# antrea-io/theia

Measured on AMD Instinct MI355X. Metric: flow-records/sec, higher is better.
Workload: dtype u64 (aggregates) + f64 (detectors)

## Files before the change

theia_amd/csrc/tad_capi.cpp:

```cpp
#include "tad_engine.h"

using namespace tad;
using namespace tadh;

namespace tadh {

int ensure_rcp_table(JobCtx *e, uint64_t T) {
  const uint64_t want = T + 2;
  if (want <= e->rcp_n) return TAD_OK;
  uint64_t cap = want < 1024 ? 1024 : want + want / 4;
  int rc = ensure(e, e->rcp_table, cap * sizeof(double));
  if (rc != TAD_OK) return rc;
  std::vector<double> h(cap);
  h[0] = 0.0;
  for (uint64_t i = 1; i < cap; ++i) h[i] = 1.0 / (double)i;
  HIP_TRY(e, hipMemcpyAsync(e->rcp_table.p, h.data(), cap * sizeof(double), hipMemcpyHostToDevice, e->stream));
  HIP_TRY(e, hipStreamSynchronize(e->stream));
  e->rcp_n = cap;
  return TAD_OK;
}

int ensure_key_buffers(JobCtx *e, uint64_t K) {
  int rc;
  const uint64_t k = K ? K : 1;
  if ((rc = ensure(e, e->sigma, k * sizeof(double))) != TAD_OK) return rc;
  if ((rc = ensure(e, e->n_pts, k * sizeof(uint32_t))) != TAD_OK) return rc;
  if ((rc = ensure(e, e->n_anom, k * sizeof(uint32_t))) != TAD_OK) return rc;
  if ((rc = ensure(e, e->off, (k + 1) * sizeof(unsigned long long))) != TAD_OK) return rc;
  if ((rc = ensure(e, e->scan_scratch, scan_scratch_elems(k) * sizeof(unsigned long long))) != TAD_OK) return rc;
  if ((rc = ensure(e, e->key_mean, k * sizeof(double))) != TAD_OK) return rc;
  if ((rc = ensure(e, e->key_m2, k * sizeof(double))) != TAD_OK) return rc;
  if ((rc = ensure(e, e->counters, kTailBytes)) != TAD_OK) return rc;
  return TAD_OK;
}

void emit_rows(JobCtx *e, Grid g, Lattice L, const JobParams &jp, OutRows out, uint64_t rows) {
  const int kind = jp.algo == TAD_ALGO_EWMA ? 0 : (jp.algo == TAD_ALGO_ARIMA ? 1 : (jp.algo == TAD_ALGO_DROP ? 3 : (jp.lazy_sigma ? 4 : 2)));
  if (kind == 4 && !jp.all_points &&
      launch_emit_dbscan_list(e->stream, g, L, e->aux.p, static_cast<const uint32_t *>(e->n_anom.p), static_cast<const unsigned long long *>(e->off.p), out))
    return;
  launch_emit(e->stream, g, L, kind, jp.all_points, jp.alpha, static_cast<const double *>(e->sigma.p),
              static_cast<const uint32_t *>(e->n_pts.p), static_cast<const double *>(kind == 3 ? e->key_mean.p : e->calc.p),
              static_cast<const unsigned long long *>(e->off.p), out, rows, e->plan.ewma_emit, e->plan.ewma_emit_rows);
}

int make_result(JobCtx *e, uint64_t rows, bool with_anomaly, tad_mem out_memory, ResultPriv **out, OutRows *dev_rows,
                ResultBlock *dev_block) {
  ResultPriv *rp = new (std::nothrow) ResultPriv();
  if (!rp) return fail(e, TAD_ERR_OUT_OF_MEMORY, "out of host memory");
  memset(rp, 0, sizeof *rp);
  const size_t bytes = result_bytes(rows, with_anomaly);
  int rc = alloc_device_block(e, bytes, dev_block);
  if (rc != TAD_OK) { delete rp; return rc; }
  carve(dev_block->base, rows, with_anomaly, dev_rows);
  rp->pub.n_rows = rows;
  rp->pub.memory = out_memory;
  *out = rp;
  return TAD_OK;
}

int finish_result(JobCtx *e, ResultPriv *rp, uint64_t rows, bool with_anomaly, ResultBlock dev_block, OutRows dev_rows) {
  if (rp->pub.memory == TAD_MEM_DEVICE) {
    rp->block = dev_block.base;
    rp->block_cap = dev_block.cap;
    rp->pub.key_id = reinterpret_cast<uint64_t *>(dev_rows.key_id);
    rp->pub.flow_end_s = reinterpret_cast<int64_t *>(dev_rows.flow_end_s);
    rp->pub.throughput = dev_rows.throughput;
    rp->pub.algo_calc = dev_rows.algo_calc;
    rp->pub.stddev = dev_rows.stddev;
    rp->pub.anomaly = dev_rows.anomaly;
    return TAD_OK;
  }
  const size_t bytes = result_bytes(rows, with_anomaly);
  void *h = malloc(bytes);
  if (!h) { release_block(e, dev_block.base, dev_block.cap); return fail(e, TAD_ERR_OUT_OF_MEMORY, "out of host memory for %zu result bytes", bytes); }
  hipError_t r = hipMemcpyAsync(h, dev_block.base, bytes, hipMemcpyDeviceToHost, e->stream);
  if (r == hipSuccess) r = hipStreamSynchronize(e->stream);
  release_block(e, dev_block.base, dev_block.cap);
  if (r != hipSuccess) { free(h); return fail(e, TAD_ERR_HIP, "result copy failed: %s", hipGetErrorString(r)); }
  OutRows ho;
  carve(h, rows, with_anomaly, &ho);
  rp->block = h;
  rp->block_cap = bytes;
  rp->pub.key_id = reinterpret_cast<uint64_t *>(ho.key_id);
  rp->pub.flow_end_s = reinterpret_cast<int64_t *>(ho.flow_end_s);
  rp->pub.throughput = ho.throughput;
  rp->pub.algo_calc = ho.algo_calc;
  rp->pub.stddev = ho.stddev;
  rp->pub.anomaly = ho.anomaly;
  return TAD_OK;
}

JobParams job_params(const tad_job *job) {
  JobParams jp;
  jp.algo = job->algo;
  jp.alpha = job->ewma_alpha == 0.0 ? 0.5 : job->ewma_alpha;
  jp.eps = job->dbscan_eps == 0.0 ? 250000000.0 : job->dbscan_eps;
  jp.min_samples = job->dbscan_min_samples == 0 ? 4 : job->dbscan_min_samples;
  jp.maxiter = job->arima_maxiter == 0 ? 50 : job->arima_maxiter;
  jp.drop_nsigma = job->drop_nsigma == 0.0 ? 3.0 : job->drop_nsigma;
  jp.drop_min_samples = job->drop_min_samples == 0 ? 3 : job->drop_min_samples;
  jp.all_points = (job->flags & TAD_FLAG_EMIT_ALL_POINTS) != 0;
  return jp;
}

void merge_moments(const Moments *blocks, bool any, double *pts_mean, double *pts_m2) {
  double mn = 0.0, mean = 0.0, m2 = 0.0;
  if (any)
    for (int b = 0; b < kMomentBlocks; ++b) {
      const Moments &p = blocks[b];
      if (p.n == 0.0) continue;
      if (mn == 0.0) { mn = p.n; mean = p.mean; m2 = p.m2; continue; }
      const double nn = mn + p.n, d = p.mean - mean;
      mean = mean + d * (p.n / nn);
      m2 = m2 + p.m2 + d * d * (mn * p.n / nn);
      mn = nn;
    }
  *pts_mean = mean;
  *pts_m2 = m2;
}

static int count_verdicts(JobCtx *e, ResultPriv *rp, uint64_t rows, uint64_t *n_anomalies) {
  *n_anomalies = 0;
  if (rows == 0) return TAD_OK;
  std::vector<uint8_t> tmp;
  const uint8_t *a = rp->pub.anomaly;
// ... 433 lines not shown
```

theia_amd/csrc/tad_capi_job.cpp:

```cpp
#include "tad_engine.h"

using namespace tad;
using namespace tadh;

namespace {

struct Job {
  const tad_job *job;
  const tad_columns *cols;
  tad_state *stream;
  bool points_mode;
  int depth;
  tad_mem out_memory;
  JobParams jp;
  tad_plan plan;
  bool op_max, has2;
  uint64_t n, K, slots_all;
  RowFilter rf;
  int cw;
  const void *d_key, *d_key2, *d_te, *d_ts, *d_val;
  DevCounters *ctr;
  bool empty;
};

struct Attempt {
  bool retry = false;
  bool finished = false;
  bool hinted = false;
  PartPlan pl{};
  Lattice L{};
  Grid g{};
  uint64_t cells = 0, need = 0;
  bool cells_overflow = false;
  bool v2 = false, sparse = false, sp_part = false, hist_sampled = false, use_kh = false, narrow_tiles = false;
  const uint32_t *binhist = nullptr;
  const unsigned long long *stream_poff = nullptr;
  uint64_t stream_P = 0;
  int stage0_path() const { return sparse ? (sp_part ? 8 : 4) : (v2 ? (pl.wc_cap ? 3 : 2) : 1); }
  int hist_source() const { return (v2 && hist_sampled) ? 1 : (use_kh ? 2 : 0); }
};

int decide(JobCtx *e, const Job &j, Stage0Retry &rs, Attempt &a, Stage0Facts f) {
  f.v2 = a.v2; f.sparse = a.sparse; f.sp_part = a.sp_part; f.use_kh = a.use_kh; f.hist_sampled = a.hist_sampled; f.narrow_tiles = a.narrow_tiles;
  const Stage0Next x = rs.next(f);
  a.retry = x.what == Stage0Next::kRetry;
  if (x.what != Stage0Next::kFail) return TAD_OK;
  if (x.code == TAD_ERR_GRID_TOO_LARGE)
    return fail(e, x.code, x.msg, (unsigned long long)a.need, (unsigned long long)j.K, (unsigned long long)a.L.nb, (long long)a.L.step, (unsigned long long)e->ws_limit);
  return fail(e, x.code, x.msg, (unsigned long long)j.K);
}

int decide(JobCtx *e, const Job &j, Stage0Retry &rs, Attempt &a, uint32_t err) {
  Stage0Facts f;
  f.err = err;
  return decide(e, j, rs, a, f);
}

int detect_and_count(JobCtx *e, Grid g, JobParams &jp, DevCounters *ctr, uint64_t *rows) {
  hipStream_t s = e->stream;
  int rc;
  if ((rc = ensure_key_buffers(e, g.K)) != TAD_OK) return rc;
  if ((rc = ensure_rcp_table(e, g.T)) != TAD_OK) return rc;
  double *sigma = static_cast<double *>(e->sigma.p);
  uint32_t *n_pts = static_cast<uint32_t *>(e->n_pts.p);
  uint32_t *n_anom = static_cast<uint32_t *>(e->n_anom.p);
  unsigned long long *off = static_cast<unsigned long long *>(e->off.p);

  const bool ewma = jp.algo == TAD_ALGO_EWMA;
  const bool drop = jp.algo == TAD_ALGO_DROP;
  const bool db_fused = jp.algo == TAD_ALGO_DBSCAN && !jp.all_points && dbscan_uses_list(g);
  jp.lazy_sigma = db_fused;
  if (drop) {
    if ((rc = ensure(e, e->calc, (g.K * g.T ? g.K * g.T : 1) * sizeof(double))) != TAD_OK) return rc;
    launch_drop(s, g, jp.drop_nsigma, jp.drop_min_samples, static_cast<double *>(e->calc.p), sigma, n_pts,
                static_cast<double *>(e->key_mean.p), static_cast<double *>(e->key_m2.p), ctr);
  } else if (!db_fused)
    launch_key_sigma(s, g, jp.alpha, ewma && !jp.all_points, static_cast<const double *>(e->rcp_table.p), sigma, n_pts, n_anom, ctr, static_cast<double *>(e->key_mean.p),
                     static_cast<double *>(e->key_m2.p));
  if (jp.algo == TAD_ALGO_DBSCAN) {
    if ((rc = ensure(e, e->aux, dbscan_scratch_bytes(g))) != TAD_OK) return rc;
    if (dbscan_uses_list(g)) {
      DbscanStats dst{nullptr, nullptr, nullptr, nullptr};
      if (db_fused) dst = DbscanStats{n_pts, n_anom, static_cast<double *>(e->key_mean.p), static_cast<double *>(e->key_m2.p)};
      if (launch_dbscan(s, g, jp.eps, jp.min_samples, e->aux.p, dst, jp.settled && db_fused) != 0)
        return fail(e, TAD_ERR_HIP, "DBSCAN launch failed");
    } else {
      return fail(e, TAD_ERR_GRID_TOO_LARGE, "DBSCAN: series of %llu buckets are not supported", (unsigned long long)g.T);
    }
  } else if (jp.algo == TAD_ALGO_ARIMA) {
    if ((rc = ensure(e, e->calc, g.K * g.T * sizeof(double))) != TAD_OK) return rc;
    const size_t wsb = arima_workspace_bytes(g);
    if ((rc = ensure(e, e->aux, wsb)) != TAD_OK) return rc;
    const bool held = e->hold && e->hold->held;
    if (held) e->hold->release();
    const unsigned int *yielded_dev = nullptr;
    if (launch_arima(s, g, sigma, n_pts, jp.maxiter, static_cast<double *>(e->calc.p), ctr, e->aux.p, wsb, e->eng->pause_dev, &yielded_dev) != 0)
      return fail(e, TAD_ERR_HIP, "ARIMA launch failed");
    if ((rc = arima_yield_loop(e, yielded_dev, [&](uint32_t grace, const unsigned int **yd) {
           return launch_arima_fit(s, g, sigma, n_pts, jp.maxiter, static_cast<double *>(e->calc.p), ctr, e->aux.p, e->eng->pause_dev, yd, grace);
         })) != TAD_OK)
      return rc;
    if (held) e->hold->acquire();
  }
  const uint32_t *cnt = n_anom;
  if (jp.all_points && jp.algo != TAD_ALGO_ARIMA && !drop) cnt = n_pts;
  else if (db_fused) {}
  else if (!ewma || jp.all_points) launch_count_flags(s, g, jp.all_points, n_anom);
  launch_scan_moments(s, cnt, off, g.K, static_cast<unsigned long long *>(e->scan_scratch.p), dev_total(e), n_pts,
                      static_cast<const double *>(e->key_mean.p), static_cast<const double *>(e->key_m2.p), dev_moments(e), db_fused ? ctr : nullptr);
  HIP_TRY(e, hipMemcpyAsync(e->tail_host, e->counters.p, kTailBytes, hipMemcpyDeviceToHost, s));
  HIP_TRY(e, hipStreamSynchronize(s));
  HIP_TRY(e, hipGetLastError());
  *rows = *e->total_host;
  return TAD_OK;
}

int stage_column(JobCtx *e, DevBuf &buf, const void *src, uint64_t n, tad_mem mem, const void **dev, uint64_t width = 8) {
  if (!src) { *dev = nullptr; return TAD_OK; }
  if (mem == TAD_MEM_DEVICE) { *dev = src; return TAD_OK; }
  int rc = ensure(e, buf, n * width);
  if (rc != TAD_OK) return rc;
  HIP_TRY(e, hipMemcpyAsync(buf.p, src, n * width, hipMemcpyHostToDevice, e->stream));
  *dev = buf.p;
  return TAD_OK;
}

int stage_columns(JobCtx *e, Job &j) {
  const tad_columns *cols = j.cols;
  const uint64_t kw = (j.cw & kColKey32) ? 4 : 8, tw = (j.cw & kColTime32) ? 4 : 8;
  int rc;
  if ((rc = stage_column(e, e->in_key, cols->key_id, j.n, cols->memory, &j.d_key, kw)) != TAD_OK) return rc;
  if ((rc = stage_column(e, e->in_key2, cols->key_id2, j.n, cols->memory, &j.d_key2, kw)) != TAD_OK) return rc;
  if ((rc = stage_column(e, e->in_te, cols->flow_end_s, j.n, cols->memory, &j.d_te, tw)) != TAD_OK) return rc;
  if ((rc = stage_column(e, e->in_ts, cols->flow_start_s, j.n, cols->memory, &j.d_ts, tw)) != TAD_OK) return rc;
  return stage_column(e, e->in_val, cols->value, j.n, cols->memory, &j.d_val);
}


int pass_a(JobCtx *e, const Job &j, const Stage0Retry &rs, Attempt &a, int *meta_blocks) {
  hipStream_t s = e->stream;
  int rc;
  const uint64_t n = j.n, K = j.K;
  a.v2 = !j.empty && j.plan.stage0 != 1 && !rs.v1 && (j.plan.stage0 == 2 || n >= (1ull << 22)) && part_plan_bins(n, K, j.has2, &a.pl);
  if (a.v2 && e->hold) e->hold->acquire();
  if ((rc = ensure(e, e->meta, sizeof(MetaPartial) * kMetaBlocks)) != TAD_OK) return rc;
  *meta_blocks = 0;
  if (!a.v2) return TAD_OK;
  const PartPlan &pl = a.pl;
  const tad_key_hist *kh = j.cols->key_hist;
  a.use_kh = j.depth == 0 && !rs.kh_rejected && kh != nullptr && kh->bins != nullptr && rs.lat_mode != 2 && kh->n_rows == n && kh->num_keys == K &&
             kh->sides == (j.has2 ? 2u : 1u) && kh->workgroups == (uint32_t)pl.G && kh->nbins == pl.nbins && kh->shift == (uint32_t)pl.shift_bin &&
             kh->chunk_rows == pl.chunk && j.rf.end_time == 0 && !(j.d_ts != nullptr && j.rf.start_time != 0);
  if ((rc = ensure(e, e->binhist, (size_t)pl.G * pl.nbins * 4)) != TAD_OK) return rc;
  a.hist_sampled = launch_meta_hist(s, (const uint64_t *)j.d_key, (const uint64_t *)j.d_key2, (const int64_t *)j.d_te, (const int64_t *)j.d_ts, n, K, j.rf,
                                    pl, static_cast<MetaPartial *>(e->meta.p), static_cast<uint32_t *>(e->binhist.p), j.ctr, j.cw,
                                    a.use_kh ||
                                    (!rs.exact_hist && rs.lat_mode != 2 && sampled_slots_bound(j.slots_all, pl) < (1ull << 32) &&
                                        (j.plan.histogram == 2 ||
                                         j.slots_all / ((uint64_t)pl.G * ((K >> kSampleBlockShift) ? (K >> kSampleBlockShift) : 1)) >= 384)));
  *meta_blocks = pl.G;
  a.binhist = static_cast<const uint32_t *>(e->binhist.p);
// ... 200 lines not shown
                                 reinterpret_cast<const uint32_t *>(ss.uval), a.L.t0, a.g, static_cast<long long *>(e->sp_times.p));
    else
      launch_sparse_place(s, ss.ucomp, ss.uval, P, static_cast<const uint32_t *>(e->sp_first.p), a.L.t0, a.g, static_cast<long long *>(e->sp_times.p));
  }
  HIP_TRY(e, hipEventRecord(e->ev[3], s));
  return TAD_OK;
}

int stage0_sparse(JobCtx *e, const Job &j, Stage0Retry &rs, Attempt &a, tad_result **out, tad_points **points_out) {
  SparseSort ss;
  int rc;
  if ((rc = sparse_sort(e, j, rs, a, ss)) != TAD_OK || a.retry) return rc;
  if (j.stream) return sparse_stream_offsets(e, j, a, ss);
  return sparse_rank_grid(e, j, rs, a, ss, out, points_out);
}

int settle_setup(JobCtx *e, Job &j, const Stage0Retry &rs, Attempt &a, SettleArgs *settle, uint32_t **ovf_keys) {
  hipStream_t s = e->stream;
  const Grid g = a.g;
  int rc;
  *settle = SettleArgs{};
  *ovf_keys = nullptr;
  j.jp.settled = false;
  if (!(j.jp.algo == TAD_ALGO_DBSCAN && !j.jp.all_points && !j.points_mode && !j.stream && dbscan_uses_list(g) &&
        part_plan_settle(a.L.nb, &a.pl, j.op_max && !rs.wide_tiles)))
    return TAD_OK;
  if ((rc = ensure(e, e->aux, dbscan_scratch_bytes(g))) != TAD_OK) return rc;
  if ((rc = ensure(e, e->ovf_keys, ((size_t)(j.K + 31) / 32) * 4 + 64)) != TAD_OK) return rc;
  *ovf_keys = static_cast<uint32_t *>(e->ovf_keys.p);
  HIP_TRY(e, hipMemsetAsync(*ovf_keys, 0, ((size_t)(j.K + 31) / 32) * 4, s));
  unsigned int *cnt = static_cast<unsigned int *>(e->aux.p);
  HIP_TRY(e, hipMemsetAsync(cnt, 0, 2 * sizeof(unsigned int), s));
  settle->redo_list = dbscan_redo_list(g, e->aux.p);
  settle->redo_count = cnt + 1;
  settle->st = DbscanStats{static_cast<uint32_t *>(e->n_pts.p), static_cast<uint32_t *>(e->n_anom.p), static_cast<double *>(e->key_mean.p),
                           static_cast<double *>(e->key_m2.p)};
  settle->list = reinterpret_cast<uint32_t *>(static_cast<unsigned char *>(e->aux.p) + 64);
  settle->count = cnt;
  settle->eps = j.jp.eps;
  settle->min_samples = j.jp.min_samples;
  settle->on = 1;
  settle->ovf_keys = *ovf_keys;
  dbscan_compact_series(g, e->aux.p, &settle->cs_val, &settle->cs_flag, &settle->cs_has, &settle->cs_cap);
  dbscan_redo_series(g, e->aux.p, &settle->rs_val, &settle->rs_flag, &settle->rs_has, &settle->rs_cap);
  j.jp.settled = true;
  a.narrow_tiles = a.pl.narrow;
  return TAD_OK;
}

int stage0_tiles(JobCtx *e, Job &j, Stage0Retry &rs, Attempt &a) {
  hipStream_t s = e->stream;
  const uint64_t n = j.n, K = j.K;
  PartPlan &pl = a.pl;
  int rc;
  part_plan_wc(a.hist_sampled ? sampled_slots_bound(j.slots_all, pl) : j.slots_all, columns_aligned16(j.d_key, j.d_key2, j.d_te, j.d_val), j.has2, j.plan.partition_pass, &pl);
  const uint64_t slots = a.hist_sampled ? sampled_slots_bound(j.slots_all, pl) : j.slots_all + pl.pad_slots;
  {
    Stage0Facts f;
    f.sampled_slots_2_32 = a.hist_sampled && slots >= (1ull << 32);
    if ((rc = decide(e, j, rs, a, f)) != TAD_OK || a.retry) return rc;
  }
  uint32_t *fin = nullptr;
  if (a.hist_sampled) {
    if ((rc = ensure(e, e->part_fin, (size_t)pl.G * pl.nparts * 8)) != TAD_OK) return rc;
    fin = static_cast<uint32_t *>(e->part_fin.p);
  }
  if ((rc = ensure(e, e->part_total, (size_t)pl.nparts * 4)) != TAD_OK) return rc;
  if ((rc = ensure(e, e->part_start, ((size_t)pl.nparts + 1) * 8)) != TAD_OK) return rc;
  if ((rc = ensure(e, e->part_offs32, (size_t)pl.G * pl.nparts * 4)) != TAD_OK) return rc;
  if ((rc = ensure(e, e->recs, (size_t)slots * 8)) != TAD_OK) return rc;
  if ((rc = ensure(e, e->ovf, 16 + (size_t)kOverflowCap * sizeof(OverflowRec))) != TAD_OK) return rc;
  unsigned long long *ovf_count = dev_ovf_count(e);
  OverflowRec *ovf = reinterpret_cast<OverflowRec *>(static_cast<unsigned char *>(e->ovf.p) + 16);
  if ((rc = ensure_key_buffers(e, K)) != TAD_OK) return rc;
  if ((rc = ensure_rcp_table(e, a.L.nb)) != TAD_OK) return rc;
  uint32_t *offs32 = static_cast<uint32_t *>(e->part_offs32.p);
  unsigned long long *part_start = static_cast<unsigned long long *>(e->part_start.p);
  if ((rc = ensure(e, e->slices, slice_table_bytes(slots, pl))) != TAD_OK) return rc;
  launch_part_offsets(s, a.binhist, pl, offs32, static_cast<uint32_t *>(e->part_total.p), part_start,
                      a.hist_sampled, static_cast<const MetaPartial *>(e->meta.p), n, slots, e->slices.p, a.g, j.ctr);
  SettleArgs settle;
  uint32_t *ovf_keys;
  if ((rc = settle_setup(e, j, rs, a, &settle, &ovf_keys)) != TAD_OK) return rc;
  HIP_TRY(e, hipEventRecord(e->ev[2], s));
  launch_partition(s, (const uint64_t *)j.d_key, (const uint64_t *)j.d_key2, (const int64_t *)j.d_te, (const int64_t *)j.d_ts,
                   (const uint64_t *)j.d_val, n, K, j.rf, a.L, pl, offs32, part_start, e->recs.p, ovf, ovf_count, kOverflowCap, j.ctr, fin, ovf_keys, j.cw);
  HIP_TRY(e, hipEventRecord(e->ev[3], s));
  launch_tile_aggregate(s, e->recs.p, part_start, pl, slots, e->slices.p, a.g, j.op_max, ovf, ovf_count, kOverflowCap,
                        a.hist_sampled ? offs32 : nullptr, fin, settle);
  return TAD_OK;
}

int stage0_dense(JobCtx *e, Job &j, Stage0Retry &rs, Attempt &a) {
  hipStream_t s = e->stream;
  const uint64_t K = j.K;
  int rc;
  if (a.cells_overflow) return fail(e, TAD_ERR_GRID_TOO_LARGE, "grid of %llu keys x %llu buckets overflows", (unsigned long long)K, (unsigned long long)a.L.nb);
  {
    Stage0Facts f;
    f.grid_too_large = a.need > e->ws_limit;
    if ((rc = decide(e, j, rs, a, f)) != TAD_OK || a.retry) return rc;
  }
  if ((rc = ensure(e, e->grid_val, a.cells * 8)) != TAD_OK) return rc;
  if ((rc = ensure(e, e->grid_flag, a.cells)) != TAD_OK) return rc;
  a.g = Grid{static_cast<unsigned long long *>(e->grid_val.p), static_cast<uint8_t *>(e->grid_flag.p), j.empty ? 0 : K, a.L.nb, nullptr};
  if (a.v2 && !part_plan_tiles(K, a.L.nb, j.has2, &a.pl)) a.v2 = false;
  if (a.v2) return stage0_tiles(e, j, rs, a);
  if (a.cells) {
    HIP_TRY(e, hipMemsetAsync(a.g.val, 0, a.cells * 8, s));
    HIP_TRY(e, hipMemsetAsync(a.g.flag, 0, a.cells, s));
  }
  HIP_TRY(e, hipEventRecord(e->ev[2], s));
  if (!j.empty)
    launch_scatter(s, (const uint64_t *)j.d_key, (const uint64_t *)j.d_key2, (const int64_t *)j.d_te, (const int64_t *)j.d_ts,
                   (const uint64_t *)j.d_val, j.n, j.rf, a.L, a.g, j.op_max, j.ctr, j.cw);
  HIP_TRY(e, hipEventRecord(e->ev[3], s));
  return TAD_OK;
}


int count_points(JobCtx *e, const Job &j, const Attempt &a, uint64_t *rows) {
  hipStream_t s = e->stream;
  const Grid g = a.g;
  int rc;
  if ((rc = ensure_key_buffers(e, g.K)) != TAD_OK) return rc;
  if ((rc = ensure_rcp_table(e, g.T)) != TAD_OK) return rc;
  launch_key_sigma(s, g, 0.5, false, static_cast<const double *>(e->rcp_table.p), static_cast<double *>(e->sigma.p),
                   static_cast<uint32_t *>(e->n_pts.p), static_cast<uint32_t *>(e->n_anom.p), j.ctr, static_cast<double *>(e->key_mean.p),
                   static_cast<double *>(e->key_m2.p));
  launch_moments(s, g.K, static_cast<const uint32_t *>(e->n_pts.p), static_cast<const double *>(e->key_mean.p),
                 static_cast<const double *>(e->key_m2.p), dev_moments(e));
  unsigned long long *off = static_cast<unsigned long long *>(e->off.p);
  launch_scan(s, static_cast<const uint32_t *>(e->n_pts.p), off, g.K, static_cast<unsigned long long *>(e->scan_scratch.p), dev_total(e));
  HIP_TRY(e, hipMemcpyAsync(e->tail_host, e->counters.p, kTailBytes, hipMemcpyDeviceToHost, s));
  HIP_TRY(e, hipStreamSynchronize(s));
  HIP_TRY(e, hipGetLastError());
  *rows = *e->total_host;
  return TAD_OK;
}

struct StreamBatches {
  HistBatch hist;
  ArimaBatch ab;
  DropBatch db;
};

int count_stream(JobCtx *e, const Job &j, const Attempt &a, StreamBatches *sb, uint64_t *rows) {
  hipStream_t s = e->stream;
  tad_state *stream = j.stream;
  const Grid g = a.g;
  const JobParams &jp = j.jp;
  const uint64_t P_bound = j.slots_all < a.cells ? j.slots_all : a.cells;
  int rc;
  if ((rc = ensure_key_buffers(e, g.K)) != TAD_OK) return rc;
  if (e->merge) {
    e->merge->changed = false;
    if (g.K && (rc = state_merge_batch(e, stream, g, a.L, a.stream_poff, a.stream_P, P_bound, j.op_max, jp.alpha, e->merge)) != TAD_OK) return rc;
  } else if (a.stream_poff)
    launch_stream_points(s, static_cast<const unsigned long long *>(e->sp_comp_a.p), static_cast<const unsigned long long *>(e->sp_val_a.p), a.stream_poff,
                         g.K, a.L.t0, jp.alpha, jp.all_points, false, state_view(stream, stream->cur), state_view(stream, stream->cur ^ 1),
                         static_cast<uint32_t *>(e->n_anom.p), nullptr, OutRows{}, j.ctr);
  else
    launch_stream(s, g, a.L, jp.alpha, jp.all_points, false, state_view(stream, stream->cur), state_view(stream, stream->cur ^ 1),
                  static_cast<uint32_t *>(e->n_anom.p), nullptr, OutRows{}, j.ctr);
  unsigned long long *off = static_cast<unsigned long long *>(e->off.p);
  if (!e->merge && (stream->history || stream->series) && g.K &&
      (rc = stream_history_batch(e, stream, g, a.L, a.stream_poff, a.stream_P, P_bound, jp, &sb->hist)) != TAD_OK)
    return rc;
  if (jp.algo == TAD_ALGO_ARIMA && g.K && (rc = stream_arima_batch(e, series_view(stream, stream->cur ^ 1), sb->hist, jp, j.ctr, &sb->ab)) != TAD_OK) return rc;
  if (jp.algo == TAD_ALGO_DROP && g.K) {
    const StateView cv = series_view(stream, stream->cur ^ 1);
    if ((rc = state_drop_batch(e, cv, sb->hist, jp, true, win_coop_min(g.K, stream->ser.len[stream->cur] + sb->hist.P_cap),
                               static_cast<uint32_t *>(e->hs_kcnt.p), reinterpret_cast<unsigned int *>(static_cast<uint32_t *>(e->hs_kcnt.p) + ((g.K + 3) & ~3ull)),
// ... 65 lines not shown
    hr = hipMemcpyAsync(h, po->d, bytes, hipMemcpyDeviceToHost, s);
  }
  if (hr == hipSuccess) hr = hipStreamSynchronize(s);
  if (hr == hipSuccess) hr = hipGetLastError();
  if (hr != hipSuccess) {
    free(h);
    drop_points(e, po);
    return fail(e, TAD_ERR_HIP, "Stage 0, points: %s", hipGetErrorString(hr));
  }
  unsigned char *base = po->d;
  if (out_memory == TAD_MEM_HOST) {
    release_block(e, po->blk.base, po->blk.cap);
    base = static_cast<unsigned char *>(h);
    pp->block = h; pp->block_cap = bytes;
  } else {
    pp->block = po->blk.base; pp->block_cap = po->blk.cap;
  }
  pp->pub.n_points = rows;
  pp->pub.key_id = reinterpret_cast<uint64_t *>(base);
  pp->pub.flow_end_s = reinterpret_cast<int64_t *>(base + po->stride * 8);
  pp->pub.value = reinterpret_cast<uint64_t *>(base + po->stride * 16);
  pp->pub.memory = out_memory;
  return TAD_OK;
}

int job_points(JobCtx *e, const Job &j, const Attempt &a, const DevCounters &c, uint64_t rows, int attempts, tad_points **points_out) {
  hipStream_t s = e->stream;
  PointsOut po;
  int rc;
  if ((rc = make_points(e, rows, &po)) != TAD_OK) return rc;
  if (rows) launch_emit_points(s, a.g, a.L, static_cast<const unsigned long long *>(e->off.p), po.key(), po.time(), po.value());
  const hipError_t er = hipEventRecord(e->ev[4], s);
  if (er != hipSuccess) { drop_points(e, &po); return fail(e, TAD_ERR_HIP, "hipEventRecord failed: %s", hipGetErrorString(er)); }
  if ((rc = finish_points(e, &po, rows, j.out_memory)) != TAD_OK) return rc;
  tad_stats &st = po.pp->pub.stats;
  stage0_stats(e, j, a, c, attempts, st);
  merge_moments(e->moments_host, a.g.K != 0, &st.pts_mean, &st.pts_m2);
  e->done.store(4);
  *points_out = &po.pp->pub;
  return TAD_OK;
}

int job_merge(JobCtx *e, const Job &j, const Attempt &a, const DevCounters &c, int attempts) {
  MergeCall *mc = e->merge;
  tad_state *stream = j.stream;
  HIP_TRY(e, hipEventRecord(e->ev[4], e->stream));
  HIP_TRY(e, hipStreamSynchronize(e->stream));
  tad_merge_stats &ms = mc->stats;
  ms.rows_in = j.n;
  ms.rows_used = c.rows_used;
  ms.stage0_path = a.stage0_path();
  ms.stage0_attempts = attempts;
  ms.job_context = e->index;
  hipEventElapsedTime(&ms.ms_stage0, e->ev[1], e->ev[5]);
  hipEventElapsedTime(&ms.ms_merge, e->ev[5], e->ev[4]);
  hipEventElapsedTime(&ms.ms_total, e->ev[0], e->ev[4]);
  if (mc->changed) state_commit(stream, stream->ser.len[stream->cur] + mc->added, stream->hist.len[stream->cur] + mc->added);
  if (j.depth == 0) e->done.store(4);
  return TAD_OK;
}

int job_rows(JobCtx *e, const Job &j, const Attempt &a, const StreamBatches &sb, const DevCounters &c, uint64_t rows, int attempts, tad_result **out) {
  hipStream_t s = e->stream;
  tad_state *stream = j.stream;
  const JobParams &jp = j.jp;
  const Grid g = a.g;
  RowsOut ro;
  int rc;
  if ((rc = make_result(e, rows, jp.all_points, j.out_memory, &ro.rp, &ro.dev_rows, &ro.dev_block)) != TAD_OK) return rc;
  if (rows && stream && jp.algo != TAD_ALGO_EWMA)
    emit_point_rows(s, jp, sb.hist, sb.ab, sb.db, state_view(stream, stream->cur ^ 1), ro.dev_rows);
  else if (rows && stream && a.stream_poff)
    launch_stream_points(s, static_cast<const unsigned long long *>(e->sp_comp_a.p), static_cast<const unsigned long long *>(e->sp_val_a.p), a.stream_poff,
                         g.K, a.L.t0, jp.alpha, jp.all_points, true, state_view(stream, stream->cur), state_view(stream, stream->cur ^ 1),
                         nullptr, static_cast<const unsigned long long *>(e->off.p), ro.dev_rows, j.ctr);
  else if (rows && stream)
    launch_stream(s, g, a.L, jp.alpha, jp.all_points, true, state_view(stream, stream->cur), state_view(stream, stream->cur ^ 1),
                  nullptr, static_cast<const unsigned long long *>(e->off.p), ro.dev_rows, j.ctr);
  else if (rows)
    emit_rows(e, g, a.L, jp, ro.dev_rows, rows);
  if ((rc = finish_rows(e, j.job, &ro, rows, jp.all_points, c, g.K != 0)) != TAD_OK) return rc;
  tad_stats &st = ro.rp->pub.stats;
  stage0_stats(e, j, a, c, attempts, st);
  st.host_syncs = (a.hinted || j.empty) ? 2 : 3;
  if (stream && g.K) {
    unsigned long long added = 0;
    memcpy(&added, e->tail_host + kTailHistLen, 8);
    state_commit(stream, stream->ser.len[stream->cur] + added, stream->hist.len[stream->cur] + added);
  }
  if (j.depth == 0) e->done.store(4);
  *out = &ro.rp->pub;
  return TAD_OK;
}

}

namespace tadh {

int run_job_locked(JobCtx *e, const tad_job *job, const tad_columns *cols, tad_mem out_memory, tad_result **out, tad_points **points_out,
                   tad_state *stream, int depth) {
  HIP_TRY(e, hipSetDevice(e->device));
  hipStream_t s = e->stream;
  if (depth == 0) {
    e->done.store(0);
    e->total.store(4);
    e->arima_relaunches = 0;
  }
  Job j{};
  j.job = job; j.cols = cols; j.stream = stream; j.points_mode = points_out != nullptr; j.depth = depth; j.out_memory = out_memory;
  j.jp = job_params(job);
  j.plan = e->plan;
  j.op_max = job->value_op == TAD_OP_MAX || (job->value_op == TAD_OP_AUTO && job->agg_flow == TAD_AGG_NONE);
  j.has2 = cols->key_id2 != nullptr;
  j.n = cols->n_rows;
  j.K = cols->num_keys;
  j.slots_all = j.n * (j.has2 ? 2 : 1);
  j.rf = RowFilter{job->start_time, job->end_time};
  j.cw = ((job->flags & TAD_FLAG_KEY_U32) ? kColKey32 : 0) | ((job->flags & TAD_FLAG_TIME_U32) ? kColTime32 : 0);
  j.empty = (j.n == 0 || j.K == 0);
  int rc;
  if ((rc = stage_columns(e, j)) != TAD_OK) return rc;
  if ((rc = ensure(e, e->counters, kTailBytes)) != TAD_OK) return rc;
  j.ctr = static_cast<DevCounters *>(e->counters.p);
  HIP_TRY(e, hipEventRecord(e->ev[0], s));
  if (depth == 0) HIP_TRY(e, hipEventRecord(e->ev[6], s));

  const Stage0Shape shape{j.n, j.K, j.has2, (int)job->algo, (int)j.op_max};
  Stage0Retry rs = Stage0Retry::start(j.plan, cols->n_buckets > 0, depth == 0 ? &e->learnt : nullptr, shape);
  for (int attempt = 1; attempt <= kStage0MaxAttempts; ++attempt) {
    Attempt a;
    HIP_TRY(e, hipMemsetAsync(j.ctr, 0, kTailMoments, s));
    j.jp.settled = false;
    if ((rc = derive_lattice(e, j, rs, a)) != TAD_OK) return rc;
    if (a.retry) continue;
    if ((rc = choose_stage0(e, j, rs, a)) != TAD_OK) return rc;
    if (a.retry) continue;
    rc = a.sparse ? stage0_sparse(e, j, rs, a, out, points_out) : stage0_dense(e, j, rs, a);
    if (rc != TAD_OK || a.finished) return rc;
    if (a.retry) continue;
    HIP_TRY(e, hipEventRecord(e->ev[5], s));
    if (depth == 0) e->done.store(2);

    uint64_t rows = 0;
    StreamBatches sb;
    if (j.points_mode) rc = count_points(e, j, a, &rows);
    else if (stream) rc = count_stream(e, j, a, &sb, &rows);
    else rc = detect_and_count(e, a.g, j.jp, j.ctr, &rows);
    if (rc != TAD_OK) return rc;
    const DevCounters c = *e->ctr_host;
    if ((rc = decide(e, j, rs, a, c.err)) != TAD_OK) return rc;
    if (a.retry) continue;
    if (depth == 0) e->done.store(3);

    if (j.points_mode) return job_points(e, j, a, c, rows, attempt, points_out);
    if (e->merge) return job_merge(e, j, a, c, attempt);
    if ((rc = job_rows(e, j, a, sb, c, rows, attempt, out)) != TAD_OK) return rc;
    if (depth == 0 && !stream) rs.learn(j.plan, shape, &e->learnt);
    return TAD_OK;
  }
  return fail(e, TAD_ERR_HIP, "internal error: Stage 0 did not settle on a lattice / strategy after %d attempts", kStage0MaxAttempts);
}

int validate_job_columns(tad_engine *e, const tad_job *job, const tad_columns *cols, const char *who) {
  if (job->agg_flow < TAD_AGG_NONE || job->agg_flow > TAD_AGG_EXTERNAL)
    return fail(e, TAD_ERR_INVALID_ARGUMENT, "invalid request: Throughput Anomaly Detector aggregated flow type should be 'pod' or 'external' or 'svc'");
  if (job->start_time != 0 && job->end_time != 0 && job->end_time <= job->start_time)
    return fail(e, TAD_ERR_INVALID_ARGUMENT, "invalid request: EndInterval should be after StartInterval");
  if (cols->n_rows > 0 && (!cols->key_id || !cols->flow_end_s || !cols->value))
    return fail(e, TAD_ERR_INVALID_ARGUMENT, "%s: key_id, flow_end_s and value columns are required", who);
  if (cols->n_rows > 0 && cols->num_keys == 0)
    return fail(e, TAD_ERR_INVALID_ARGUMENT, "%s: num_keys is 0 but there are rows", who);
  if ((job->flags & TAD_FLAG_KEY_U32) && cols->num_keys >= 0xFFFFFFFFull)
    return fail(e, TAD_ERR_INVALID_ARGUMENT, "%s: TAD_FLAG_KEY_U32 needs num_keys < 2^32 - 1 (TAD_KEY_SKIP32 is the skip marker)", who);
  if (cols->n_buckets > 0 && cols->step < 1)
    return fail(e, TAD_ERR_INVALID_ARGUMENT, "%s: lattice hint needs step >= 1", who);
  return TAD_OK;
}

}

namespace {

int run_job(tad_engine *eng, const tad_job *job, const tad_columns *cols, tad_mem out_memory, tad_result **out, tad_points **points_out,
            tad_state *stream = nullptr) {
  tad_engine *e = eng;
  const bool points_mode = points_out != nullptr;
  if (stream && e && job && cols) {
    if (job->algo == TAD_ALGO_DBSCAN && !stream->history)
      return fail(e, TAD_ERR_INVALID_ARGUMENT, "tad_run_stream: DBSCAN needs a state with history (tad_state_create_ex with TAD_STATE_HISTORY)");
    if (job->algo == TAD_ALGO_ARIMA && !stream->series)
      return fail(e, TAD_ERR_INVALID_ARGUMENT, "tad_run_stream: ARIMA needs a state with a series (tad_state_create_ex with TAD_STATE_SERIES)");
    if (job->algo != TAD_ALGO_EWMA && job->algo != TAD_ALGO_DBSCAN && job->algo != TAD_ALGO_ARIMA)
      return fail(e, TAD_ERR_INVALID_ARGUMENT, "tad_run_stream: only the EWMA detector has a streaming form, DBSCAN on a state with history and "
                                               "ARIMA on a state with a series (DROP: tad_drop_stream)");
    if (cols->num_keys != stream->K) return fail(e, TAD_ERR_INVALID_ARGUMENT, "tad_run_stream: batch declares %llu keys, the state holds %llu (they must be equal)",
                                                 (unsigned long long)cols->num_keys, (unsigned long long)stream->K);
  }
  if (!e) return fail(nullptr, TAD_ERR_INVALID_ARGUMENT, "tad_run: engine is NULL");
  if (!job || !cols || (!out && !points_out)) return fail(e, TAD_ERR_INVALID_ARGUMENT, "tad_run: job, cols and out must not be NULL");
  if (out) *out = nullptr;
  if (points_out) *points_out = nullptr;
  if (!points_mode && job->algo != TAD_ALGO_EWMA && job->algo != TAD_ALGO_ARIMA && job->algo != TAD_ALGO_DBSCAN && job->algo != TAD_ALGO_DROP)
    return fail(e, TAD_ERR_INVALID_ARGUMENT, "invalid request: Throughput Anomaly Detector algorithm type should be 'EWMA' or 'ARIMA' or 'DBSCAN'");
  {
    const int vrc = validate_job_columns(e, job, cols, "tad_run");
    if (vrc != TAD_OK) return vrc;
  }
  if (job->ewma_alpha < 0.0 || job->ewma_alpha > 1.0 || job->dbscan_eps < 0.0 || job->dbscan_min_samples < 0 || job->arima_maxiter < 0 ||
      job->drop_nsigma < 0.0 || job->drop_min_samples < 0)
    return fail(e, TAD_ERR_INVALID_ARGUMENT, "tad_run: detector parameter out of range");

  std::unique_lock<std::mutex> state_lk;
  if (stream) state_lk = std::unique_lock<std::mutex>(stream->mu);
  if (stream && stream->times_stale)
    return fail(e, TAD_ERR_INVALID_ARGUMENT, "tad_run_stream: the series was imported without its times (tad_state_import_times); state unchanged");
  Lease lease(eng, job->id, !points_mode && job->algo == TAD_ALGO_ARIMA);
  if (!lease.c) return fail(eng, TAD_ERR_OUT_OF_MEMORY, "tad_run: no job context available");
  PauseHold hold(eng);
  lease.c->hold = &hold;
  return run_job_locked(lease.c, job, cols, out_memory, out, points_out, stream, 0);
}

int sparse_points_direct(JobCtx *e, uint64_t n_rows_in, uint64_t rows_used, Lattice L, uint64_t P, DevCounters *ctr, tad_mem out_memory,
                         tad_points **points_out) {
  hipStream_t s = e->stream;
  int rc;
  if ((rc = ensure(e, e->counters, kTailBytes)) != TAD_OK) return rc;
  PointsOut po;
  if ((rc = make_points(e, P, &po)) != TAD_OK) return rc;
  launch_sparse_points_out(s, static_cast<const unsigned long long *>(e->sp_comp_a.p), static_cast<const unsigned long long *>(e->sp_val_a.p), P, L.t0,
// ... 177 lines not shown
```

theia_amd/csrc/tad_engine.h:

```cpp
#ifndef THEIA_TAD_ENGINE_H
#define THEIA_TAD_ENGINE_H

#include <atomic>
#include <chrono>
#include <condition_variable>
#include <cstdarg>
#include <cstdio>
#include <cstdlib>
#include <cstring>
#include <mutex>
#include <new>
#include <optional>
#include <string>
#include <thread>
#include <utility>
#include <vector>

#include "tad_internal.h"
#include "tad_stage0_retry.h"

struct DevBuf {
  void *p = nullptr;
  size_t cap = 0;
};
// ... 195 lines not shown
    }
    c->busy = true;
    c->plan = eng->plan;
    c->done.store(0);
    c->total.store(0);
    memset(c->id, 0, sizeof c->id);
    if (id) strncpy(c->id, id, sizeof c->id - 1);
    c->stream = low_priority ? c->stream_low : c->stream_normal;
    c->hold = nullptr;
  }
  ~Lease() {
    if (!c) return;
    {
      std::lock_guard<std::mutex> lk(eng->mu);
      if (c->total.load() != 0) { eng->last_done = c->done.load(); eng->last_total = c->total.load(); }
      c->busy = false;
      c->id[0] = 0;
      c->hold = nullptr;
    }
    eng->cv.notify_one();
  }
  Lease(const Lease &) = delete;
  Lease &operator=(const Lease &) = delete;
};


struct StateCall {
  tad_engine *eng;
  std::unique_lock<std::mutex> state_lk;
  std::optional<Lease> lease;
  JobCtx *e = nullptr;
  StateCall(tad_engine *eng_, const tad_state *st) : eng(eng_), state_lk(st->mu) {}
  int enter(const char *who, const char *id = nullptr, bool low_priority = false) {
    lease.emplace(eng, id, low_priority);
    e = lease->c;
    if (!e) return fail(eng, TAD_ERR_OUT_OF_MEMORY, "%s: no job context available", who);
    HIP_TRY(e, hipSetDevice(e->device));
    return TAD_OK;
  }
};

void release_block(tad_engine *eng, void *p, size_t cap);
inline void release_block(JobCtx *e, void *p, size_t cap) { release_block(e->eng, p, cap); }

Lattice make_lattice(int64_t t0, int64_t step, uint64_t nb);
uint64_t host_gcd(uint64_t a, uint64_t b);

struct ResultBlock {
  void *base = nullptr;
  size_t cap = 0;
};

size_t result_bytes(uint64_t rows, bool with_anomaly);
void carve(void *base, uint64_t rows, bool with_anomaly, OutRows *o);
int alloc_device_block(JobCtx *e, size_t bytes, ResultBlock *rb);

struct ResultPriv {
  tad_result pub;
  void *block;
  size_t block_cap;
};

struct PointsPriv {
  tad_points pub;
  void *block;
  size_t block_cap;
};

struct DropRowsPriv {
  tad_drop_rows pub;
  void *block;
  size_t block_cap;
};

struct JobParams {
  tad_algo algo;
  double alpha, eps;
  int min_samples, maxiter;
  double drop_nsigma;
  int drop_min_samples;
  bool all_points;
  bool lazy_sigma = false;
  bool settled = false;
};

int ensure_rcp_table(JobCtx *e, uint64_t T);
int ensure_key_buffers(JobCtx *e, uint64_t K);
void emit_rows(JobCtx *e, Grid g, Lattice L, const JobParams &jp, OutRows out, uint64_t rows = 0);

JobParams job_params(const tad_job *job);
void merge_moments(const Moments *blocks, bool any, double *pts_mean, double *pts_m2);
struct RowsOut {
  ResultPriv *rp = nullptr;
  OutRows dev_rows{};
  ResultBlock dev_block;
};
int make_result(JobCtx *e, uint64_t rows, bool with_anomaly, tad_mem out_memory, ResultPriv **out, OutRows *dev_rows, ResultBlock *dev_block);
int finish_result(JobCtx *e, ResultPriv *rp, uint64_t rows, bool with_anomaly, ResultBlock dev_block, OutRows dev_rows);
int finish_rows(JobCtx *e, const tad_job *job, RowsOut *ro, uint64_t rows, bool with_anomaly, const DevCounters &c, bool any_points);

struct HistBatch {
  const unsigned long long *nk = nullptr, *nv = nullptr;
  const long long *nt = nullptr;
  const unsigned long long *poff = nullptr;
  const unsigned long long *P_dev = nullptr;
  uint64_t P_cap = 0;
  const uint8_t *noise = nullptr;
  const uint32_t *cnt = nullptr;
  const unsigned long long *row = nullptr;
};
struct ArimaBatch {
  uint64_t P = 0;
  const unsigned long long *tidx = nullptr;
  const double *sigma = nullptr;
  const double *pcalc = nullptr;
  const uint8_t *pflag = nullptr;
  const uint32_t *rows = nullptr;
  const unsigned long long *row_off = nullptr;
};
struct DropBatch {
  DropStateKeys keys{};
  const uint8_t *flag = nullptr;
  const uint32_t *cnt = nullptr;
  const unsigned long long *row = nullptr;
};
int hist_verdicts(JobCtx *e, const unsigned long long *hoff, const unsigned long long *hval, const JobParams &jp, HistBatch *hb);
void emit_point_rows(hipStream_t s, const JobParams &jp, const HistBatch &hb, const ArimaBatch &ab, const DropBatch &db, const StreamState &mom,
                     OutRows out);
int stream_history_batch(JobCtx *e, tad_state *st, Grid g, Lattice L, const unsigned long long *sparse_poff, uint64_t P, uint64_t P_bound,
                         const JobParams &jp, HistBatch *hb);
int state_merge_batch(JobCtx *e, tad_state *st, Grid g, Lattice L, const unsigned long long *sparse_poff, uint64_t P, uint64_t P_bound, bool op_max,
                      double alpha, MergeCall *mc);
int stream_arima_batch(JobCtx *e, const StateView &v, const HistBatch &hb, const JobParams &jp, DevCounters *ctr, ArimaBatch *ab);
int state_drop_batch(JobCtx *e, const StateView &v, const HistBatch &hb, const JobParams &jp, bool touched_only, unsigned long long coop_min,
                     uint32_t *list, unsigned int *lcount, DevCounters *ctr, DropBatch *db);

int run_job_locked(JobCtx *e, const tad_job *job, const tad_columns *cols, tad_mem out_memory, tad_result **out, tad_points **points_out,
                   tad_state *stream, int depth);
int validate_job_columns(tad_engine *e, const tad_job *job, const tad_columns *cols, const char *who);

template <typename Relaunch>
int arima_yield_loop(JobCtx *e, const unsigned int *yielded_dev, Relaunch relaunch) {
  hipStream_t s = e->stream;
  while (yielded_dev != nullptr && e->eng->pause_dev != nullptr) {
    unsigned int y = 0;
    HIP_TRY(e, hipMemcpyAsync(&y, yielded_dev, 4, hipMemcpyDeviceToHost, s));
    HIP_TRY(e, hipStreamSynchronize(s));
    if (y == 0) break;
    const auto t0 = std::chrono::steady_clock::now();
    while (__atomic_load_n(&e->eng->pause_count, __ATOMIC_ACQUIRE) != 0 && std::chrono::steady_clock::now() - t0 < std::chrono::milliseconds(2))
      std::this_thread::sleep_for(std::chrono::microseconds(50));
    const uint32_t grace = __atomic_load_n(&e->eng->pause_count, __ATOMIC_ACQUIRE) != 0 ? 24u : 0u;
    if (relaunch(grace, &yielded_dev) != 0) return fail(e, TAD_ERR_HIP, "ARIMA launch failed");
    e->arima_relaunches++;
  }
  return TAD_OK;
}

size_t state_bytes(uint64_t K);
StreamState stream_view(void *block, uint64_t K);
StreamState state_view(const tad_state *st, int which);
StateView series_view(const tad_state *st, int which);
int state_grow_candidates(JobCtx *e, tad_state *st, uint64_t P_cap);
void state_commit(tad_state *st, uint64_t n_ser, uint64_t n_hist);
uint64_t state_device_bytes(const tad_state *st);

// ... 4 lines not shown
```

theia_amd/csrc/tad_internal.h:

```cpp
#pragma once
#include <hip/hip_runtime.h>
#include <stdint.h>
#include <type_traits>

#include "tad.h"
#include "tad_dev_err.h"

namespace tad {

struct Lattice {
  int64_t t0;
  int64_t step;
  uint64_t nb;
  uint64_t magic;
  int mode;
};

struct Grid {
  unsigned long long *val;
  uint8_t *flag;
  uint64_t K;
  uint64_t T;
  const long long *times;
};

enum : uint8_t { FLAG_PRESENT = 1, FLAG_ANOMALY = 2 };

struct MetaPartial {
  int64_t tmin, tmax, tref;
  uint64_t g;
  uint64_t used;
  uint64_t seen;
};

struct DevCounters {
  unsigned long long rows_used;
  unsigned long long n_keys;
  unsigned long long n_points;
  unsigned long long keys_no_result;
  unsigned long long kalman_steps;
  unsigned long long arima_fits;
  unsigned long long arima_nan_fits;
  uint32_t err;
  uint32_t pad;
};

enum : int { kColKey32 = 1, kColTime32 = 2 };

struct RowFilter {
  int64_t start_time;
  int64_t end_time;
};

struct OutRows {
  unsigned long long *key_id;
  long long *flow_end_s;
  double *throughput;
  double *algo_calc;
  double *stddev;
  uint8_t *anomaly;
};

inline void allow_big_lds(const void *kernel, size_t bytes) {
  hipFuncSetAttribute(kernel, hipFuncAttributeMaxDynamicSharedMemorySize, (int)bytes);
}

int launch_meta(hipStream_t s, const uint64_t *key, const uint64_t *key2, const int64_t *t_end,
                const int64_t *t_start, uint64_t n, RowFilter f, MetaPartial *partials, int n_blocks, int cw = 0);

void launch_scatter(hipStream_t s, const uint64_t *key, const uint64_t *key2, const int64_t *t_end,
                    const int64_t *t_start, const uint64_t *value, uint64_t n, RowFilter f,
                    Lattice lat, Grid g, bool op_max, DevCounters *ctr, int cw = 0);

__device__ __forceinline__ double div_by_count(double a, double b, double y) {
  double q = a * y;
  double r = fma(-b, q, a);
  q = fma(r, y, q);
  r = fma(-b, q, a);
  return fma(r, y, q);
}

struct Moments { double n, mean, m2; };

#if defined(__HIPCC__)
__device__ __forceinline__ uint64_t key_of32(uint32_t v) { return v == 0xFFFFFFFFu ? TAD_KEY_SKIP : (uint64_t)v; }
template <bool K32> __device__ __forceinline__ uint64_t ld_key(const uint64_t *p, uint64_t i) {
  if constexpr (K32) return key_of32(reinterpret_cast<const uint32_t *>(p)[i]);
  else return p[i];
}
template <bool T32> __device__ __forceinline__ int64_t ld_time(const int64_t *p, uint64_t i) {
  if constexpr (T32) return (int64_t)(uint64_t)reinterpret_cast<const uint32_t *>(p)[i];
  else return p[i];
}
template <bool K32> __device__ __forceinline__ ulonglong2 ld_key2(const uint64_t *p, uint64_t base, uint64_t j) {
  if constexpr (K32) { const uint2 v = reinterpret_cast<const uint2 *>(reinterpret_cast<const uint32_t *>(p) + base)[j]; return make_ulonglong2(key_of32(v.x), key_of32(v.y)); }
  else return reinterpret_cast<const ulonglong2 *>(p + base)[j];
}
template <bool T32> __device__ __forceinline__ longlong2 ld_time2(const int64_t *p, uint64_t base, uint64_t j) {
  if constexpr (T32) { const uint2 v = reinterpret_cast<const uint2 *>(reinterpret_cast<const uint32_t *>(p) + base)[j]; return make_longlong2((int64_t)v.x, (int64_t)v.y); }
  else return reinterpret_cast<const longlong2 *>(p + base)[j];
}
template <typename F> inline void with_widths(int cw, F &&f) {
  switch (cw & (kColKey32 | kColTime32)) {
    case 0: f(std::false_type{}, std::false_type{}); break;
    case kColKey32: f(std::true_type{}, std::false_type{}); break;
    case kColTime32: f(std::false_type{}, std::true_type{}); break;
    default: f(std::true_type{}, std::true_type{}); break;
  }
}

static constexpr int kWalkChunk = 8;

template <typename Step>
__device__ __forceinline__ void walk_series(const Grid &g, uint64_t k, Step step) {
  const uint64_t T = g.T;
  const uint64_t nfull = T / kWalkChunk;
  uint8_t fa[kWalkChunk], fb[kWalkChunk];
  unsigned long long va[kWalkChunk], vb[kWalkChunk];
  auto load = [&](uint64_t c, uint8_t *f, unsigned long long *v) {
#pragma unroll
    for (int u = 0; u < kWalkChunk; ++u) {
      const uint64_t cell = (c * kWalkChunk + u) * g.K + k;
      f[u] = g.flag[cell];
      v[u] = g.val[cell];
    }
  };
  if (nfull) {
    load(0, fa, va);
    uint64_t c = 0;
    for (; c + 2 <= nfull; c += 2) {
      load(c + 1, fb, vb);
#pragma unroll
      for (int u = 0; u < kWalkChunk; ++u) step(c * kWalkChunk + u, fa[u], va[u]);
      load(c + 2 < nfull ? c + 2 : c + 1, fa, va);
#pragma unroll
      for (int u = 0; u < kWalkChunk; ++u) step((c + 1) * kWalkChunk + u, fb[u], vb[u]);
    }
    if (c < nfull) {
#pragma unroll
      for (int u = 0; u < kWalkChunk; ++u) step(c * kWalkChunk + u, fa[u], va[u]);
    }
  }
  for (uint64_t t = nfull * kWalkChunk; t < T; ++t) step(t, g.flag[t * g.K + k], g.val[t * g.K + k]);
}

static constexpr uint64_t kCoopMinT = 512, kCoopMaxK = 8192;
inline bool coop_shape(const Grid &g) { return g.T >= kCoopMinT && g.K <= kCoopMaxK; }

__device__ __forceinline__ uint32_t readlane_u32(uint32_t v, int l) { return (uint32_t)__builtin_amdgcn_readlane((int)v, l); }
__device__ __forceinline__ double readlane_f64(double v, int l) {
  const unsigned long long b = (unsigned long long)__double_as_longlong(v);
  const unsigned long long r = ((unsigned long long)readlane_u32((uint32_t)(b >> 32), l) << 32) | readlane_u32((uint32_t)b, l);
  return __longlong_as_double((long long)r);
}

template <typename Block, typename Step>
__device__ __forceinline__ void walk_series_coop(const Grid &g, uint64_t k, Block block, Step step) {
  const uint64_t T = g.T;
  const unsigned lane = threadIdx.x & 63u;
  const uint64_t nblk = (T + 63) / 64;
  auto load = [&](uint64_t c, uint32_t &f, unsigned long long &v) {
    const uint64_t t = c * 64 + lane;
    const bool in = c < nblk && t < T;
    f = in ? (uint32_t)g.flag[t * g.K + k] : 0u;
    v = in ? g.val[t * g.K + k] : 0ull;
  };
  uint32_t f0, f1, f2;
  unsigned long long v0, v1, v2;
  load(0, f0, v0);
  load(1, f1, v1);
  for (uint64_t c = 0; c < nblk; ++c) {
    load(c + 2, f2, v2);
    const uint64_t t0 = c * 64;
    const double x0 = (double)v0;
    const unsigned long long present = __ballot((f0 & FLAG_PRESENT) != 0);
    block(c);
    int ord = 0;
    for (unsigned long long m = present; m; m &= m - 1, ++ord) {
      const int u = __ffsll((long long)m) - 1;
      step(t0 + (uint64_t)u, (uint8_t)readlane_u32(f0, u), readlane_f64(x0, u), ord);
    }
    f0 = f1; v0 = v1;
    f1 = f2; v1 = v2;
  }
}

__device__ __forceinline__ Moments chan_merge(Moments a, Moments b) {
  if (b.n == 0.0) return a;
  if (a.n == 0.0) return b;
  Moments r;
  r.n = a.n + b.n;
  const double d = b.mean - a.mean;
  r.mean = a.mean + d * (b.n / r.n);
  r.m2 = a.m2 + b.m2 + d * d * (a.n * b.n / r.n);
  return r;
}

#endif

void launch_key_sigma(hipStream_t s, Grid g, double alpha, bool ewma_count, const double *rcp, double *sigma,
                      uint32_t *n_pts, uint32_t *n_anom, DevCounters *ctr, double *key_mean, double *key_m2);
static constexpr int kMomentBlocks = 128;
void launch_moments(hipStream_t s, uint64_t K, const uint32_t *n_pts, const double *key_mean,
                    const double *key_m2, Moments *partials, DevCounters *ctr = nullptr);
void launch_count_flags(hipStream_t s, Grid g, bool all_points, uint32_t *n_anom);
void launch_scan(hipStream_t s, const uint32_t *cnt, unsigned long long *off, uint64_t K,
                 unsigned long long *scratch, unsigned long long *total_copy = nullptr);
size_t scan_scratch_elems(uint64_t K);
void launch_scan_moments(hipStream_t s, const uint32_t *cnt, unsigned long long *off, uint64_t K, unsigned long long *scratch,
                         unsigned long long *total_copy, const uint32_t *n_pts, const double *key_mean, const double *key_m2, Moments *partials,
                         DevCounters *ctr);
void launch_emit(hipStream_t s, Grid g, Lattice lat, int kind, bool all_points, double alpha,
                 const double *sigma, const uint32_t *n_pts, const double *calc,
                 const unsigned long long *off, OutRows out, uint64_t rows_hint = 0,
                 int ewma_emit = 0, uint32_t ewma_emit_rows = 0);
void launch_emit_points(hipStream_t s, Grid g, Lattice lat, const unsigned long long *off, unsigned long long *out_key,
                        long long *out_t, unsigned long long *out_val);
struct StreamState {
  uint32_t *n;
  double *avg, *m2, *ewma;
  long long *last_t;
  unsigned char *seen;
};
struct StreamAcc {
  uint32_t n;
  double cnt, avg, m2, e;
  long long last_t;
  bool seen;
};

__device__ __forceinline__ StreamAcc stream_load(const StreamState &cur, uint64_t k) {
  const uint32_t n = cur.n[k];
  return StreamAcc{n, (double)n, cur.avg[k], cur.m2[k], cur.ewma[k], cur.last_t[k], cur.seen[k] != 0};
}

__device__ __forceinline__ void stream_store(const StreamState &next, uint64_t k, const StreamAcc &a) {
  next.n[k] = a.n; next.avg[k] = a.avg; next.m2[k] = a.m2; next.ewma[k] = a.e; next.last_t[k] = a.last_t; next.seen[k] = a.seen ? 1 : 0;
}

__device__ __forceinline__ bool stream_step(StreamAcc &a, double alpha, double one_minus, double x, long long ts, double *sg) {
  a.cnt = a.cnt + 1.0;
  a.n++;
  const double d = x - a.avg;
  const double dn = d / a.cnt;
  a.avg = a.avg + dn;
  a.m2 = a.m2 + d * (d - dn);
  a.e = one_minus * a.e + alpha * x;
  const bool has_sigma = a.n >= 2;
  *sg = has_sigma ? sqrt(a.m2 / (a.cnt - 1.0)) : 0.0;
  a.last_t = ts;
  a.seen = true;
  return has_sigma && fabs(x - a.e) > *sg;
}

void launch_stream(hipStream_t s, Grid g, Lattice lat, double alpha, bool all_points, bool emit, StreamState cur, StreamState next,
                   uint32_t *n_anom, const unsigned long long *off, OutRows out, DevCounters *ctr);
void launch_stream_points(hipStream_t s, const unsigned long long *comp, const unsigned long long *val, const unsigned long long *poff, uint64_t K,
                          int64_t t0, double alpha, bool all_points, bool emit, StreamState cur, StreamState next, uint32_t *n_anom,
                          const unsigned long long *off, OutRows out, DevCounters *ctr);
void launch_hist_decode(hipStream_t s, const unsigned long long *comp, uint64_t P, int64_t t0, unsigned long long *nk, long long *nt);
void launch_hist_sort(hipStream_t s, const unsigned long long *nv, const unsigned long long *poff, uint64_t K, unsigned long long *ns,
                      uint32_t *long_list, unsigned int *long_count);
static constexpr uint32_t kHistChunk = 2048;
#if defined(__HIPCC__)
__device__ __forceinline__ uint64_t chunk_key(const unsigned long long *coff, uint64_t K, unsigned long long w) {
  uint64_t lo = 0, hi = K;
  while (hi - lo > 1) { const uint64_t mid = (lo + hi) >> 1; if (coff[mid] <= w) lo = mid; else hi = mid; }
  return lo;
}
__device__ __forceinline__ uint64_t chunk_key_min1(const unsigned long long *coff, uint64_t K, unsigned long long w) {
  return coff[K] == K ? w : chunk_key(coff, K, w);
}
#endif
uint64_t hist_merge_chunks_bound(uint64_t K, uint64_t total_len);
void launch_hist_merge(hipStream_t s, uint64_t K, const unsigned long long *hoff_old, const unsigned long long *hval_old, const unsigned long long *poff,
                       const unsigned long long *ns, unsigned long long *hoff_new, unsigned long long *hval_new, uint32_t *chunks,
                       unsigned long long *coff, unsigned long long *scan_scratch, uint64_t chunks_bound);
void launch_hist_verdict(hipStream_t s, const unsigned long long *nk, const unsigned long long *nv, const unsigned long long *P_dev, uint64_t P_cap,
                         const unsigned long long *hoff, const unsigned long long *h, double eps, int min_samples, bool all_points, uint8_t *noise,
                         uint32_t *cnt);
void launch_hist_emit(hipStream_t s, const unsigned long long *nk, const long long *nt, const unsigned long long *nv, const unsigned long long *P_dev,
                      uint64_t P_cap, const uint8_t *noise, const uint32_t *cnt, const unsigned long long *row, StreamState next, bool all_points,
                      OutRows out);
void launch_ewma_values(hipStream_t s, Grid g, double alpha, double *calc);

struct DbscanStats {
  uint32_t *n_pts, *n_anom;
  double *key_mean, *key_m2;
};
struct SettleArgs {
  DbscanStats st;
  uint32_t *list;
  unsigned int *count;
  double eps;
  int32_t min_samples;
  uint32_t on;
  unsigned long long *cs_val;
  uint8_t *cs_flag;
// ... 90 lines not shown
void launch_as_touch(hipStream_t s, uint64_t K, const unsigned long long *soff, const unsigned long long *poff, uint32_t *touched, uint32_t *len8,
                     unsigned int *tmax);
void launch_as_prep(hipStream_t s, uint64_t K, const unsigned long long *soff, const unsigned long long *sval, const unsigned long long *poff,
                    StreamState next, const unsigned long long *tidx, const unsigned long long *yoffk, double *lx, double *ysk, ArimaSlots sl,
                    double *pcalc, uint8_t *pflag, DevCounters *ctr);
void launch_as_list(hipStream_t s, uint64_t Kt, ArimaSlots sl, bool fill, unsigned int *cnt, const unsigned long long *loff, uint32_t *list, uint32_t *fpos);
size_t arima_stream_ws_bytes(uint64_t nfits, uint64_t npos, uint64_t waves);
int launch_arima_stream_fit(hipStream_t s, bool first, uint64_t nfits, uint64_t npos, uint64_t waves, const uint32_t *fpos, double *ysk,
                            ArimaSlots sl, FitListArgs fa, int maxiter, DevCounters *ctr, void *workspace, const int *pause,
                            const unsigned int **yielded, uint32_t grace);
void launch_as_rows(hipStream_t s, uint64_t P, const unsigned long long *nk, const unsigned long long *tidx, const uint8_t *ok, const uint8_t *pflag,
                    bool all_points, uint32_t *rows);
void launch_as_emit(hipStream_t s, uint64_t P, const unsigned long long *nk, const long long *nt, const unsigned long long *nv,
                    const unsigned long long *tidx, const double *sigma, const double *pcalc, const uint8_t *pflag, const uint32_t *rows,
                    const unsigned long long *row_off, bool all_points, OutRows out);
void launch_drop(hipStream_t s, Grid g, double n_sigma, int min_samples, double *ws, double *sigma, uint32_t *n_pts,
                 double *key_mean, double *key_m2, DevCounters *ctr);

struct DropStateKeys {
  double *mean, *std, *m2;
  uint32_t *n;
  uint8_t *ok;
};
size_t drop_state_key_bytes(uint64_t K);
DropStateKeys drop_state_keys(void *mem, uint64_t K);
void launch_ds_route(hipStream_t s, uint64_t K, const unsigned long long *soff, const unsigned long long *poff, unsigned long long coop_min, uint32_t *list,
                     unsigned int *count);
void launch_ds_stats(hipStream_t s, uint64_t K, const unsigned long long *soff, const unsigned long long *sval, const unsigned long long *poff,
                     unsigned long long coop_min, const uint32_t *list, const unsigned int *count, int min_samples, DropStateKeys d, DevCounters *ctr);
void launch_ds_verdict(hipStream_t s, const unsigned long long *nk, const unsigned long long *nv, const unsigned long long *P_dev, uint64_t P_cap,
                       DropStateKeys d, double n_sigma, bool all_points, uint8_t *flag, uint32_t *cnt);
void launch_ds_emit(hipStream_t s, const unsigned long long *nk, const long long *nt, const unsigned long long *nv, const unsigned long long *P_dev,
                    uint64_t P_cap, const uint8_t *flag, const uint32_t *cnt, const unsigned long long *row, DropStateKeys d, bool all_points, OutRows out);

int launch_arima(hipStream_t s, Grid g, const double *sigma, const uint32_t *n_pts, int maxiter,
                 double *calc, DevCounters *ctr, void *workspace, size_t workspace_bytes, const int *pause = nullptr, const unsigned int **yielded = nullptr);
int launch_arima_fit(hipStream_t s, Grid g, const double *sigma, const uint32_t *n_pts, int maxiter, double *calc, DevCounters *ctr, void *workspace,
                     const int *pause, const unsigned int **yielded, uint32_t grace);
size_t arima_workspace_bytes(Grid g);

struct OverflowRec {
  unsigned long long val;
  unsigned long long gcell;
};
constexpr uint32_t kMaxBins = 16384;
struct PartPlan {
  int shift_bin;
  uint32_t nbins;
  int G;
  uint64_t chunk;
  int shift_part;
  uint32_t KP, nparts, bins_per_part;
  size_t agg_lds, part_lds;
  int rpt;
  int cell_bits;
  uint32_t tb, n_chunks;
  uint32_t settle_kt;
  bool narrow;
  uint32_t wc_cap;
  uint32_t wc_sec, wc_rpt;
  uint64_t pad_slots;
  int sp_tbits;
};
void part_plan_wc(uint64_t slots, bool aligned, bool has2, int partition_pass, PartPlan *pl);
bool columns_aligned16(const void *key, const void *key2, const void *t_end, const void *value);
bool part_plan_bins(uint64_t n, uint64_t K, bool has2, PartPlan *pl);
bool part_plan_tiles(uint64_t K, uint64_t T, bool has2, PartPlan *pl);
bool part_plan_sparse(uint64_t K, uint64_t T, bool has2, PartPlan *pl);
bool launch_meta_hist(hipStream_t s, const uint64_t *key, const uint64_t *key2, const int64_t *t_end,
                      const int64_t *t_start, uint64_t n, uint64_t K, RowFilter f, const PartPlan &pl,
                      MetaPartial *partials, uint32_t *binhist, DevCounters *ctr, int cw, bool sample_hist);
void launch_part_offsets(hipStream_t s, const uint32_t *binhist, const PartPlan &pl, uint32_t *offs32, uint32_t *total,
                         unsigned long long *part_start, bool sampled, const MetaPartial *partials, uint64_t n, uint64_t slots, void *slice_mem,
                         Grid g, DevCounters *ctr = nullptr);
uint64_t sampled_slots_bound(uint64_t slots, const PartPlan &pl);
void launch_partition(hipStream_t s, const uint64_t *key, const uint64_t *key2, const int64_t *t_end,
                      const int64_t *t_start, const uint64_t *value, uint64_t n, uint64_t K, RowFilter f,
                      Lattice L, const PartPlan &pl, const uint32_t *offs32, const unsigned long long *part_start,
                      void *recs, OverflowRec *ovf, unsigned long long *ovf_count, uint32_t ovf_cap, DevCounters *ctr,
                      uint32_t *fin = nullptr, uint32_t *ovf_keys = nullptr, int cw = 0);
size_t slice_table_bytes(uint64_t slots, const PartPlan &pl);
void launch_tile_aggregate(hipStream_t s, const void *recs, const unsigned long long *part_start, const PartPlan &pl,
                           uint64_t slots, void *slice_mem, Grid g, bool op_max, const OverflowRec *ovf,
                           const unsigned long long *ovf_count, uint32_t ovf_cap, const uint32_t *offs32, const uint32_t *fin, SettleArgs settle);
bool part_plan_settle(uint64_t T, PartPlan *pl, bool narrow = false);

size_t sparse_sort_temp_bytes(uint64_t slots);
size_t sparse_part_temp_bytes(const PartPlan &pl);
void launch_sparse_sort(hipStream_t s, const void *recs, const unsigned long long *part_start, const uint32_t *binhist, const PartPlan &pl, uint64_t K,
                        int64_t step, bool op_max, unsigned long long *recs2, unsigned long long *stage_comp, unsigned long long *stage_val,
                        uint32_t *stage_rank, void *temp, unsigned long long *num_runs, DevCounters *ctr);
void launch_sparse_place_staged(hipStream_t s, const PartPlan &pl, void *temp, const unsigned long long *stage_comp, const unsigned long long *stage_val,
                                const uint32_t *stage_rank, int64_t t0, Grid g, long long *times);
void launch_sparse_compact(hipStream_t s, const PartPlan &pl, void *temp, const unsigned long long *stage_comp, const unsigned long long *stage_val,
                           unsigned long long *comp_out, unsigned long long *val_out);
int launch_sparse_group(hipStream_t s, const uint64_t *key, const uint64_t *key2, const int64_t *t_end, const int64_t *t_start,
                        const uint64_t *value, uint64_t n, uint64_t K, RowFilter f, int64_t t0, uint64_t span, bool op_max, unsigned long long *comp_a,
                        unsigned long long *val_a, unsigned long long *comp_b, unsigned long long *val_b, void *temp, size_t temp_bytes,
                        unsigned long long *num_runs, DevCounters *ctr, int cw = 0);
void launch_sparse_tmax(hipStream_t s, const unsigned long long *ucomp, uint64_t slots, const unsigned long long *P_dev, uint32_t *first, unsigned int *tmax);
void launch_sparse_place(hipStream_t s, const unsigned long long *ucomp, const unsigned long long *uval, uint64_t P, const uint32_t *first,
                         int64_t t0, Grid g, long long *times);
uint32_t sparse_class_count(uint32_t tmax);
void launch_sparse_len(hipStream_t s, const unsigned long long *ucomp, uint64_t P, const uint32_t *first, uint32_t *len);
void launch_sparse_class_counts(hipStream_t s, const uint32_t *len, uint64_t K, uint32_t c, uint32_t *member, uint32_t *pts);
void launch_sparse_class_columns(hipStream_t s, const unsigned long long *ucomp, const unsigned long long *uval, uint64_t P, const uint32_t *first,
                                 const uint32_t *len, uint32_t c, const unsigned long long *key_off, const unsigned long long *pt_off, int64_t t0,
                                 unsigned long long *out_key, long long *out_t, unsigned long long *out_val, uint32_t *keymap);
void launch_sparse_points_out(hipStream_t s, const unsigned long long *ucomp, const unsigned long long *uval, uint64_t P, int64_t t0,
                              unsigned long long *out_key, long long *out_t, unsigned long long *out_val, Moments *partials, DevCounters *ctr);
void launch_class_count_rows(hipStream_t s, const unsigned long long *row_key, uint64_t R, const uint32_t *keymap, uint32_t *cnt,
                             unsigned long long *first_row);
void launch_class_gather(hipStream_t s, OutRows src, uint64_t R, const uint32_t *keymap, const unsigned long long *off,
                         const unsigned long long *first_row, OutRows dst);


bool shard_world_ok(uint32_t world);
void launch_shard_count(hipStream_t s, const uint64_t *key, uint64_t n, uint32_t world, unsigned long long *counts);
void launch_shard_scatter(hipStream_t s, const uint64_t *key, const int64_t *t_end, const uint64_t *value, uint64_t n, uint32_t world,
                          unsigned long long *cursor, uint64_t *out_key, int64_t *out_t, uint64_t *out_val);

static constexpr int kFzMaxCols = 8;
uint64_t factorize_table_slots(uint64_t virtual_rows);
uint64_t factorize_first_slots(uint64_t virtual_rows);
uint64_t factorize_next_slots(uint64_t virtual_rows, uint64_t slots);
size_t factorize_temp_bytes(uint64_t virtual_rows, uint64_t slots);
void launch_factorize(hipStream_t s, const long long *const *cols_a, const uint8_t *keep_a, const long long *const *cols_b, const uint8_t *keep_b, uint64_t n,
                      int n_cols, uint64_t slots, void *temp, uint64_t *key_a, uint64_t *key_b, uint64_t *first_row, uint64_t first_row_cap,
                      unsigned long long *num_keys_dev, uint32_t **flags_dev_out, uint32_t *hist_bins = nullptr, int hist_workgroups = 0, uint64_t hist_chunk = 0);
void launch_encode_strings(hipStream_t s, const void *offsets, int off64, const uint8_t *data, uint64_t data_bytes, const uint8_t *valid, uint64_t valid_off,
                           uint64_t n, uint64_t slots, void *temp, long long *codes, uint64_t *first_row, uint64_t first_row_cap,
                           unsigned long long *num_values_dev, uint32_t **flags_dev_out, const uint8_t *keep = nullptr);

struct KdBatch {
  const long long *a[kFzMaxCols];
  const long long *b[kFzMaxCols];
  const uint8_t *keep_a, *keep_b;
  uint64_t n;
  int n_cols;
  uint32_t sides;
};
static constexpr uint32_t kKdMaxProbe = 32;
enum : uint32_t { KD_FLAG_CLUSTER = 1u, KD_FLAG_DUPLICATE = 2u, KD_FLAG_BAD_ROW = 4u, KD_FLAG_BAD_CODE = 8u };
int kd_stride(int n_cols);
void launch_kd_probe(hipStream_t s, const KdBatch &A, const unsigned long long *table, uint64_t slots, const unsigned long long *keys, uint64_t K, uint64_t *key_a,
                     uint64_t *key_b, uint8_t *miss, unsigned long long *n_miss);
void launch_kd_append(hipStream_t s, const KdBatch &A, const uint64_t *first_row, uint64_t m, uint64_t K0, unsigned long long *table, uint64_t slots,
                      unsigned long long *keys, uint32_t *flags);
void launch_kd_fix(hipStream_t s, const uint8_t *miss, const uint64_t *loc_a, const uint64_t *loc_b, uint64_t n, uint32_t sides, uint64_t K0, uint64_t *key_a,
                   uint64_t *key_b);
void launch_kd_rehash(hipStream_t s, const unsigned long long *keys, int n_cols, uint64_t K, unsigned long long *table, uint64_t slots, uint32_t *flags,
                      bool check_duplicates);
static constexpr int kKdMaxTerms = 8;
struct KdSelect {
  const uint8_t *mask[kKdMaxTerms];
  unsigned long long mask_len[kKdMaxTerms];
  int32_t col[kKdMaxTerms];
  int32_t n_terms, side;
};
void launch_kd_select(hipStream_t s, const unsigned long long *keys, int n_cols, uint64_t K, const KdSelect &q, uint8_t *keep, unsigned long long *n_sel,
                      uint32_t *flags);

struct SdBatch {
  const void *offsets;
  const uint8_t *data;
  const uint8_t *valid;
  uint64_t valid_off, n, data_bytes;
// ... 77 lines not shown
```

theia_amd/csrc/tad_kernels.hip:

```cpp
#include <cstdlib>

#include "tad_internal.h"

namespace tad {

static constexpr int kBlock = 256;

__device__ __forceinline__ uint64_t gcd_u64(uint64_t a, uint64_t b) {
  if (a == 0) return b;
  if (b == 0) return a;
  if (((a | b) >> 32) == 0) {
    uint32_t x = (uint32_t)a, y = (uint32_t)b;
    while (y) { uint32_t r = x % y; x = y; y = r; }
    return x;
  }
  while (b) { uint64_t r = a % b; a = b; b = r; }
  return a;
}

__device__ __forceinline__ uint64_t absdiff_i64(int64_t a, int64_t b) {
  return a >= b ? (uint64_t)a - (uint64_t)b : (uint64_t)b - (uint64_t)a;
}

struct MetaAcc {
// ... 103 lines not shown
template <bool OPMAX>
__device__ __forceinline__ void scatter_row(uint64_t k1, uint64_t k2, bool has2, int64_t te, uint64_t v,
                                            const Lattice &L, const Grid &g, uint32_t &err, uint32_t &used) {
  uint64_t bucket;
  const bool live1 = k1 != TAD_KEY_SKIP, live2 = has2 && k2 != TAD_KEY_SKIP;
  if (!live1 && !live2) return;
  if (!cell_index(L, te, bucket)) { err |= DEV_ERR_OFF_LATTICE; return; }
  if (live1) {
    if (k1 >= g.K) err |= DEV_ERR_KEY_RANGE;
    else { cell_update<OPMAX>(g, bucket, k1, v); used++; }
  }
  if (live2) {
    if (k2 >= g.K) err |= DEV_ERR_KEY_RANGE;
    else { cell_update<OPMAX>(g, bucket, k2, v); used++; }
  }
}

template <bool OPMAX, bool VEC2, bool K32 = false, bool T32 = false>
__global__ __launch_bounds__(kBlock) void k_scatter(const uint64_t *__restrict__ key,
                                                    const uint64_t *__restrict__ key2,
                                                    const int64_t *__restrict__ t_end,
                                                    const int64_t *__restrict__ t_start,
                                                    const uint64_t *__restrict__ value, uint64_t n,
                                                    RowFilter f, Lattice L, Grid g, DevCounters *ctr) {
  uint32_t err = 0, used = 0;
  const uint64_t stride = (uint64_t)gridDim.x * kBlock;
  const uint64_t tid = (uint64_t)blockIdx.x * kBlock + threadIdx.x;
  const bool has2 = key2 != nullptr;
  if (VEC2) {
    const uint64_t n2 = n >> 1;
    const ulonglong2 *val_v = reinterpret_cast<const ulonglong2 *>(value);
    for (uint64_t i = tid; i < n2; i += stride) {
      const ulonglong2 k = ld_key2<K32>(key, 0, i);
      const longlong2 te = ld_time2<T32>(t_end, 0, i);
      const ulonglong2 v = val_v[i];
      ulonglong2 k2 = make_ulonglong2(TAD_KEY_SKIP, TAD_KEY_SKIP);
      if (has2) k2 = ld_key2<K32>(key2, 0, i);
      if (row_kept<T32>(te.x, t_start, 2 * i, f)) scatter_row<OPMAX>(k.x, k2.x, has2, te.x, v.x, L, g, err, used);
      if (row_kept<T32>(te.y, t_start, 2 * i + 1, f)) scatter_row<OPMAX>(k.y, k2.y, has2, te.y, v.y, L, g, err, used);
    }
    if ((n & 1) && tid == 0) {
      const uint64_t i = n - 1;
      if (row_kept<T32>(ld_time<T32>(t_end, i), t_start, i, f))
        scatter_row<OPMAX>(ld_key<K32>(key, i), has2 ? ld_key<K32>(key2, i) : TAD_KEY_SKIP, has2, ld_time<T32>(t_end, i), value[i], L, g, err, used);
    }
  } else {
    for (uint64_t i = tid; i < n; i += stride) {
      if (row_kept<T32>(ld_time<T32>(t_end, i), t_start, i, f))
        scatter_row<OPMAX>(ld_key<K32>(key, i), has2 ? ld_key<K32>(key2, i) : TAD_KEY_SKIP, has2, ld_time<T32>(t_end, i), value[i], L, g, err, used);
    }
  }
  unsigned long long u = used;
  for (int d = 32; d >= 1; d >>= 1) {
    u += __shfl_down(u, d);
    err |= __shfl_down(err, d);
  }
  if ((threadIdx.x & 63) == 0) {
    if (u) atomicAdd(&ctr->rows_used, u);
    if (err) atomicOr(&ctr->err, err);
  }
}

void launch_scatter(hipStream_t s, const uint64_t *key, const uint64_t *key2, const int64_t *t_end,
                    const int64_t *t_start, const uint64_t *value, uint64_t n, RowFilter f,
                    Lattice lat, Grid g, bool op_max, DevCounters *ctr, int cw) {
  if (n == 0) return;
  auto aligned16 = [](const void *p) { return p == nullptr || (reinterpret_cast<uintptr_t>(p) & 15) == 0; };
  const bool vec = aligned16(key) && aligned16(key2) && aligned16(t_end) && aligned16(value) && n >= 2;
  const uint64_t work = vec ? (n >> 1) : n;
  int blocks = (int)((work + kBlock - 1) / kBlock);
  if (blocks > 256 * 16) blocks = 256 * 16;
  if (blocks < 1) blocks = 1;
  with_widths(cw, [&](auto k32, auto t32) {
#define TAD_LAUNCH_SCATTER(OPMAX, VEC) \
  hipLaunchKernelGGL((k_scatter<OPMAX, VEC, k32(), t32()>), dim3(blocks), dim3(kBlock), 0, s, key, key2, t_end, t_start, value, n, f, lat, g, ctr)
    if (op_max) { if (vec) TAD_LAUNCH_SCATTER(true, true); else TAD_LAUNCH_SCATTER(true, false); }
    else        { if (vec) TAD_LAUNCH_SCATTER(false, true); else TAD_LAUNCH_SCATTER(false, false); }
#undef TAD_LAUNCH_SCATTER
  });
}

static constexpr int kUnroll = 16;

template <bool EWMA_COUNT, bool RCP_LDS, bool COOP = false>
__global__ __launch_bounds__(kBlock) void k_key_sigma(Grid g, double alpha, const double *__restrict__ rcp_g, double *__restrict__ sigma,
                                                      uint32_t *__restrict__ n_pts,
                                                      uint32_t *__restrict__ n_anom, DevCounters *ctr,
                                                      double *__restrict__ key_mean, double *__restrict__ key_m2) {
  const uint64_t gtid = (uint64_t)blockIdx.x * kBlock + threadIdx.x;
  const uint64_t k = COOP ? gtid >> 6 : gtid;
  const bool writer = !COOP || (threadIdx.x & 63) == 0;
  extern __shared__ __attribute__((aligned(16))) unsigned char smem_rcp[];
  const double *rcp = rcp_g;
  if (RCP_LDS) {
    double *l = reinterpret_cast<double *>(smem_rcp);
    for (uint64_t i = threadIdx.x; i <= g.T; i += kBlock) l[i] = rcp_g[i];
    __syncthreads();
    rcp = l;
  }
  unsigned long long my_pts = 0;
  unsigned my_key = 0;
  if (k < g.K) {
    double cnt = 0.0, avg = 0.0, m2 = 0.0;
    uint32_t n = 0;
    auto sigma_step = [&](uint64_t, uint8_t fl, unsigned long long raw) {
      if (fl & FLAG_PRESENT) {
        const double x = (double)raw;
        cnt = cnt + 1.0;
        n++;
        const double d = x - avg;
        const double dn = RCP_LDS ? div_by_count(d, cnt, rcp[n]) : d / cnt;
        avg = avg + dn;
        m2 = m2 + d * (d - dn);
      }
    };
    if (COOP) {
      double rl = 0.0;
      walk_series_coop(g, k,
                       [&](uint64_t) { rl = 1.0 / (double)(n + 1u + (threadIdx.x & 63u)); },
                       [&](uint64_t, uint8_t, double x, int ord) {
                         cnt = cnt + 1.0;
                         n++;
                         const double d = x - avg;
                         const double dn = div_by_count(d, cnt, readlane_f64(rl, ord));
                         avg = avg + dn;
                         m2 = m2 + d * (d - dn);
                       });
    } else {
      walk_series(g, k, sigma_step);
    }
    const bool has_sigma = n >= 2;
    const double sg = has_sigma ? sqrt(m2 / (cnt - 1.0)) : 0.0;
    if (writer) {
      sigma[k] = sg;
      n_pts[k] = n;
      if (key_mean != nullptr) { key_mean[k] = avg; key_m2[k] = m2; }
      my_pts = n;
      my_key = n > 0;
    }
    if (EWMA_COUNT) {
      uint32_t a = 0;
      if (has_sigma) {
        const double one_minus = 1.0 - alpha;
        double e = 0.0;
        auto ewma_step = [&](uint64_t, uint8_t fl, unsigned long long raw) {
          if (fl & FLAG_PRESENT) {
            const double x = (double)raw;
            e = one_minus * e + alpha * x;
            a += fabs(x - e) > sg ? 1u : 0u;
          }
        };
        if (COOP) walk_series_coop(g, k, [](uint64_t) {}, [&](uint64_t, uint8_t, double x, int) {
                    e = one_minus * e + alpha * x;
                    a += fabs(x - e) > sg ? 1u : 0u;
                  });
        else walk_series(g, k, ewma_step);
      }
      if (writer) n_anom[k] = a;
    }
  }
  for (int d = 32; d >= 1; d >>= 1) {
    my_pts += __shfl_down(my_pts, d);
    my_key += __shfl_down(my_key, d);
  }
  if ((threadIdx.x & 63) == 0 && my_key) {
    atomicAdd(&ctr->n_points, my_pts);
    atomicAdd(&ctr->n_keys, (unsigned long long)my_key);
  }
}

void launch_key_sigma(hipStream_t s, Grid g, double alpha, bool ewma_count, const double *rcp, double *sigma,
                      uint32_t *n_pts, uint32_t *n_anom, DevCounters *ctr, double *key_mean, double *key_m2) {
  if (g.K == 0) return;
  const size_t lds = (size_t)(g.T + 1) * 8;
  const bool in_lds = lds <= 32768;
  if (coop_shape(g)) {
    const int cblocks = (int)((g.K * 64 + kBlock - 1) / kBlock);
#define TAD_KSC(EC, RL) hipLaunchKernelGGL((k_key_sigma<EC, RL, true>), dim3(cblocks), dim3(kBlock), RL ? lds : 0, s, g, alpha, rcp, sigma, n_pts, n_anom, ctr, key_mean, key_m2)
    if (ewma_count) { if (in_lds) TAD_KSC(true, true); else TAD_KSC(true, false); }
    else { if (in_lds) TAD_KSC(false, true); else TAD_KSC(false, false); }
#undef TAD_KSC
    return;
  }
  const int blocks = (int)((g.K + kBlock - 1) / kBlock);
#define TAD_KS(EC, RL) hipLaunchKernelGGL((k_key_sigma<EC, RL>), dim3(blocks), dim3(kBlock), RL ? lds : 0, s, g, alpha, rcp, sigma, n_pts, n_anom, ctr, key_mean, key_m2)
  if (ewma_count) { if (in_lds) TAD_KS(true, true); else TAD_KS(true, false); }
  else { if (in_lds) TAD_KS(false, true); else TAD_KS(false, false); }
#undef TAD_KS
}


struct MomentsArgs {
  uint64_t K;
  const uint32_t *n_pts;
  const double *key_mean, *key_m2;
  Moments *partials;
  DevCounters *ctr;
};

__device__ __forceinline__ void moments_block(uint32_t mb, uint64_t K, const uint32_t *__restrict__ n_pts,
                                              const double *__restrict__ key_mean,
                                              const double *__restrict__ key_m2,
                                              Moments *__restrict__ partials, DevCounters *ctr) {
  Moments acc{0.0, 0.0, 0.0};
  unsigned long long pts = 0, keys = 0;
  const uint64_t stride = (uint64_t)kMomentBlocks * kBlock;
  constexpr int kMU = 8;
  for (uint64_t k = (uint64_t)mb * kBlock + threadIdx.x; k < K; k += stride * kMU) {
    uint32_t n[kMU];
    double mean[kMU], m2[kMU];
#pragma unroll
    for (int u = 0; u < kMU; ++u) {
      const uint64_t ku = k + (uint64_t)u * stride;
      const bool in = ku < K;
      n[u] = in ? n_pts[ku] : 0u;
      mean[u] = in ? key_mean[ku] : 0.0;
      m2[u] = in ? key_m2[ku] : 0.0;
    }
#pragma unroll
    for (int u = 0; u < kMU; ++u) {
      acc = chan_merge(acc, Moments{(double)n[u], mean[u], m2[u]});
      pts += n[u];
      keys += n[u] > 0;
    }
  }
  if (ctr != nullptr) {
    for (int d = 32; d >= 1; d >>= 1) { pts += __shfl_down(pts, d); keys += __shfl_down(keys, d); }
    if ((threadIdx.x & 63) == 0 && keys) { atomicAdd(&ctr->n_points, pts); atomicAdd(&ctr->n_keys, keys); }
  }
  for (int d = 1; d < 64; d <<= 1) {
    Moments o{__shfl_xor(acc.n, d), __shfl_xor(acc.mean, d), __shfl_xor(acc.m2, d)};
    acc = (threadIdx.x & d) ? chan_merge(o, acc) : chan_merge(acc, o);
  }
  __shared__ Moments s_m[kBlock / 64];
  if ((threadIdx.x & 63) == 0) s_m[threadIdx.x >> 6] = acc;
  __syncthreads();
  if (threadIdx.x == 0) {
    Moments a = s_m[0];
    for (int w = 1; w < kBlock / 64; ++w) a = chan_merge(a, s_m[w]);
    partials[mb] = a;
  }
}

__global__ __launch_bounds__(kBlock) void k_moments(MomentsArgs M) {
  moments_block(blockIdx.x, M.K, M.n_pts, M.key_mean, M.key_m2, M.partials, M.ctr);
}

void launch_moments(hipStream_t s, uint64_t K, const uint32_t *n_pts, const double *key_mean,
                    const double *key_m2, Moments *partials, DevCounters *ctr) {
  hipLaunchKernelGGL(k_moments, dim3(kMomentBlocks), dim3(kBlock), 0, s, MomentsArgs{K, n_pts, key_mean, key_m2, partials, ctr});
}

__global__ __launch_bounds__(kBlock) void k_count_flags(Grid g, bool all_points, uint32_t *__restrict__ n_anom) {
  const uint64_t k = (uint64_t)blockIdx.x * kBlock + threadIdx.x;
  if (k >= g.K) return;
  const uint8_t want = all_points ? FLAG_PRESENT : (uint8_t)(FLAG_PRESENT | FLAG_ANOMALY);
  uint32_t a = 0;
  for (uint64_t t = 0; t < g.T; ++t) a += (g.flag[t * g.K + k] & want) == want ? 1u : 0u;
// ... 73 lines not shown
  if (threadIdx.x == 0) {
    *total_out = carry;
    if (total_copy != nullptr) *total_copy = carry;
  }
}

static constexpr uint64_t kScanOwnBaseBlocks = 4096;
template <bool OWN_BASE>
__global__ __launch_bounds__(kBlock) void k_scan_apply(const uint32_t *__restrict__ cnt, uint64_t K,
                                                       const unsigned long long *__restrict__ bsum,
                                                       unsigned long long *__restrict__ off, uint32_t nb, unsigned long long *total_copy) {
  const uint64_t base = (uint64_t)blockIdx.x * kScanTile + (uint64_t)threadIdx.x * kScanItems;
  uint32_t c[kScanItems];
  unsigned long long s = 0;
  for (int j = 0; j < kScanItems; ++j) {
    c[j] = base + j < K ? cnt[base + j] : 0u;
    s += c[j];
  }
  unsigned long long bbase;
  if (OWN_BASE) {
    unsigned long long before = 0, all = 0;
    for (uint32_t i = threadIdx.x; i < nb; i += kBlock) {
      const unsigned long long v = bsum[i];
      all += v;
      if (i < blockIdx.x) before += v;
    }
    unsigned long long t1, t2;
    block_exclusive_scan(before, &t1);
    block_exclusive_scan(all, &t2);
    bbase = t1;
    if (blockIdx.x == 0 && threadIdx.x == 0) {
      off[K] = t2;
      if (total_copy != nullptr) *total_copy = t2;
    }
  } else {
    bbase = bsum[blockIdx.x];
  }
  unsigned long long tot;
  unsigned long long ex = block_exclusive_scan(s, &tot) + bbase;
  for (int j = 0; j < kScanItems; ++j) {
    if (base + j < K) off[base + j] = ex;
    ex += c[j];
  }
}

size_t scan_scratch_elems(uint64_t K) { return (size_t)((K + kScanTile - 1) / kScanTile) + 1; }

static void scan_launches(hipStream_t s, const uint32_t *cnt, unsigned long long *off, uint64_t K, unsigned long long *scratch,
                          unsigned long long *total_copy, const MomentsArgs *M) {
  const uint64_t nb = (K + kScanTile - 1) / kScanTile;
  const MomentsArgs none{0, nullptr, nullptr, nullptr, nullptr, nullptr};
  if (M != nullptr) hipLaunchKernelGGL(k_scan_reduce<true>, dim3((unsigned)nb + kMomentBlocks), dim3(kBlock), 0, s, cnt, K, scratch, (uint32_t)nb, *M);
  else hipLaunchKernelGGL(k_scan_reduce<false>, dim3((unsigned)nb), dim3(kBlock), 0, s, cnt, K, scratch, (uint32_t)nb, none);
  if (nb <= kScanOwnBaseBlocks) {
    hipLaunchKernelGGL(k_scan_apply<true>, dim3((unsigned)nb), dim3(kBlock), 0, s, cnt, K, scratch, off, (uint32_t)nb, total_copy);
    return;
  }
  hipLaunchKernelGGL(k_scan_top, dim3(1), dim3(kBlock), 0, s, scratch, nb, off + K, total_copy);
  hipLaunchKernelGGL(k_scan_apply<false>, dim3((unsigned)nb), dim3(kBlock), 0, s, cnt, K, scratch, off, (uint32_t)nb, total_copy);
}

void launch_scan(hipStream_t s, const uint32_t *cnt, unsigned long long *off, uint64_t K,
                 unsigned long long *scratch, unsigned long long *total_copy) {
  if (K == 0) {
    hipMemsetAsync(off, 0, sizeof(unsigned long long), s);
    if (total_copy != nullptr) hipMemsetAsync(total_copy, 0, sizeof(unsigned long long), s);
    return;
  }
  scan_launches(s, cnt, off, K, scratch, total_copy, nullptr);
}

void launch_scan_moments(hipStream_t s, const uint32_t *cnt, unsigned long long *off, uint64_t K, unsigned long long *scratch,
                         unsigned long long *total_copy, const uint32_t *n_pts, const double *key_mean, const double *key_m2, Moments *partials,
                         DevCounters *ctr) {
  if (K == 0) {
    launch_scan(s, cnt, off, K, scratch, total_copy);
    launch_moments(s, K, n_pts, key_mean, key_m2, partials, ctr);
    return;
  }
  const MomentsArgs M{K, n_pts, key_mean, key_m2, partials, ctr};
  scan_launches(s, cnt, off, K, scratch, total_copy, &M);
}

template <int KIND, bool ALL, bool COOP = false>
__global__ __launch_bounds__(kBlock) void k_emit(Grid g, Lattice L, double alpha,
                                                 const double *__restrict__ sigma,
                                                 const uint32_t *__restrict__ n_pts,
                                                 const double *__restrict__ calc,
                                                 const unsigned long long *__restrict__ off, OutRows out) {
  const uint64_t gtid = (uint64_t)blockIdx.x * kBlock + threadIdx.x;
  const uint64_t k = COOP ? gtid >> 6 : gtid;
  const bool writer = !COOP || (threadIdx.x & 63) == 0;
  if (k >= g.K) return;
  unsigned long long pos = off[k];
  const unsigned long long end = off[k + 1];
  if (pos == end) return;
  constexpr bool LAZY = KIND == 4;
  const unsigned long long first = pos;
  double sg = LAZY ? 0.0 : sigma[k];
  double s_cnt = 0.0, s_avg = 0.0, s_m2 = 0.0;
  const bool has_sigma = n_pts[k] >= 2;
  const double one_minus = 1.0 - alpha;
  double e = 0.0;
  long long bt[4];
  double bx[4], ba[4];
  uint8_t bv[4] = {0, 0, 0, 0};
  int nb = 0;
  auto write_row = [&](unsigned long long at, long long ts, double x, double a, bool verdict) {
    if (!writer) return;
    out.key_id[at] = k;
    out.flow_end_s[at] = ts;
    out.throughput[at] = x;
    out.algo_calc[at] = a;
    if (!LAZY) out.stddev[at] = sg;
    if (ALL) out.anomaly[at] = verdict ? 1 : 0;
  };
  auto point = [&](uint64_t t, uint8_t fl, double x) {
    if (LAZY) {
      s_cnt = s_cnt + 1.0;
      const double d = x - s_avg;
      const double dn = d / s_cnt;
      s_avg = s_avg + dn;
      s_m2 = s_m2 + d * (d - dn);
    }
    double a;
    bool verdict;
    if (KIND == 0) {
      e = one_minus * e + alpha * x;
      a = e;
      verdict = has_sigma && fabs(x - e) > sg;
    } else {
      a = KIND == 1 ? calc[t * g.K + k] : (KIND == 3 ? calc[k] : 0.0);
      verdict = (fl & FLAG_ANOMALY) != 0;
    }
    if ((ALL || verdict) && pos + nb < end) {
      const long long ts = g.times != nullptr ? g.times[t * g.K + k] : (long long)(L.t0 + (int64_t)t * L.step);
      if (nb == 0 && (pos & 3ull) != 0) {
        write_row(pos, ts, x, a, verdict);
        pos++;
      } else {
#pragma unroll
        for (int i = 0; i < 4; ++i)
          if (nb == i) { bt[i] = ts; bx[i] = x; ba[i] = a; if (ALL) bv[i] = verdict ? 1 : 0; }
        if (++nb == 4 && !writer) { pos += 4; nb = 0; }
        else if (nb == 4) {
          const ulonglong2 kk = make_ulonglong2(k, k);
          reinterpret_cast<ulonglong2 *>(out.key_id + pos)[0] = kk;
          reinterpret_cast<ulonglong2 *>(out.key_id + pos)[1] = kk;
          reinterpret_cast<longlong2 *>(out.flow_end_s + pos)[0] = make_longlong2(bt[0], bt[1]);
          reinterpret_cast<longlong2 *>(out.flow_end_s + pos)[1] = make_longlong2(bt[2], bt[3]);
          reinterpret_cast<double2 *>(out.throughput + pos)[0] = make_double2(bx[0], bx[1]);
          reinterpret_cast<double2 *>(out.throughput + pos)[1] = make_double2(bx[2], bx[3]);
          reinterpret_cast<double2 *>(out.algo_calc + pos)[0] = make_double2(ba[0], ba[1]);
          reinterpret_cast<double2 *>(out.algo_calc + pos)[1] = make_double2(ba[2], ba[3]);
          if (!LAZY) {
            const double2 ss = make_double2(sg, sg);
            reinterpret_cast<double2 *>(out.stddev + pos)[0] = ss;
            reinterpret_cast<double2 *>(out.stddev + pos)[1] = ss;
          }
          if (ALL) *reinterpret_cast<uint32_t *>(out.anomaly + pos) = (uint32_t)bv[0] | ((uint32_t)bv[1] << 8) | ((uint32_t)bv[2] << 16) | ((uint32_t)bv[3] << 24);
          pos += 4;
          nb = 0;
        }
      }
    }
  };
  if (COOP) walk_series_coop(g, k, [](uint64_t) {}, [&](uint64_t t, uint8_t fl, double x, int) { point(t, fl, x); });
  else walk_series(g, k, [&](uint64_t t, uint8_t fl, unsigned long long raw) { if (fl & FLAG_PRESENT) point(t, fl, (double)raw); });
#pragma unroll
  for (int i = 0; i < 3; ++i)
    if (i < nb) write_row(pos + i, bt[i], bx[i], ba[i], ALL && bv[i] != 0);
  if (LAZY) {
    sg = has_sigma ? sqrt(s_m2 / (s_cnt - 1.0)) : 0.0;
    if (COOP) { for (unsigned long long at = first + (threadIdx.x & 63); at < end; at += 64) out.stddev[at] = sg; }
    else { for (unsigned long long at = first; at < end; ++at) out.stddev[at] = sg; }
  }
}

static constexpr int kStageMarkTBits = 26;
__global__ __launch_bounds__(64) void k_emit_staged(Grid g, Lattice L, double alpha, const double *__restrict__ sigma,
                                                    const uint32_t *__restrict__ n_pts,
                                                    const unsigned long long *__restrict__ off, OutRows out, uint32_t cap) {
  extern __shared__ __attribute__((aligned(16))) unsigned char smem_stage[];
  double *s_e = reinterpret_cast<double *>(smem_stage);
  double *s_sg = s_e + cap;
  uint32_t *s_m = reinterpret_cast<uint32_t *>(s_sg + 64);
  const uint32_t lane = threadIdx.x;
  const uint64_t k0 = (uint64_t)blockIdx.x * 64;
  const uint64_t k = k0 + lane;
  const uint64_t kend = k0 + 64 < g.K ? k0 + 64 : g.K;
  const unsigned long long base = off[k0];
  const unsigned long long total = off[kend] - base;
  if (total == 0) return;
  const bool live = k < g.K;
  unsigned long long pos = live ? off[k] - base : 0;
  const unsigned long long end = live ? off[k + 1] - base : 0;
  const double sg = live ? sigma[k] : 0.0;
  s_sg[lane] = sg;
  if (pos != end) {
    const double one_minus = 1.0 - alpha;
    double e = 0.0;
    walk_series(g, k, [&](uint64_t t, uint8_t fl, unsigned long long raw) {
      if (!(fl & FLAG_PRESENT)) return;
      const double x = (double)raw;
      e = one_minus * e + alpha * x;
      if (fabs(x - e) > sg && pos < end) {
        if (pos < cap) {
          s_e[pos] = e;
          s_m[pos] = (lane << kStageMarkTBits) | (uint32_t)t;
        } else {
          const unsigned long long at = base + pos;
          out.key_id[at] = k;
          out.flow_end_s[at] = g.times != nullptr ? g.times[t * g.K + k] : (long long)(L.t0 + (int64_t)t * L.step);
          out.throughput[at] = x;
          out.algo_calc[at] = e;
          out.stddev[at] = sg;
        }
        pos++;
      }
    });
  }
  __syncthreads();
  const unsigned long long staged = total < cap ? total : cap;
  for (unsigned long long r = lane; r < staged; r += 64) {
    const uint32_t m = s_m[r];
    const uint32_t ln = m >> kStageMarkTBits;
    const uint64_t t = m & ((1u << kStageMarkTBits) - 1u);
    const uint64_t cell = t * g.K + (k0 + ln);
    const unsigned long long at = base + r;
    out.key_id[at] = k0 + ln;
    out.flow_end_s[at] = g.times != nullptr ? g.times[cell] : (long long)(L.t0 + (int64_t)t * L.step);
    out.throughput[at] = (double)g.val[cell];
    out.algo_calc[at] = s_e[r];
    out.stddev[at] = s_sg[ln];
  }
}

static uint32_t emit_stage_rows(uint64_t K, uint64_t rows_hint, int ewma_emit, uint32_t ewma_emit_rows) {
  if (ewma_emit == 1) return 0;
  uint64_t cap = 1536;
  if (rows_hint != 0) {
    const uint64_t mean = (rows_hint * 64 + K - 1) / K;
    cap = mean + mean / 8 + 128;
  }
  if (ewma_emit_rows != 0) cap = ewma_emit_rows;
  cap = (cap + 63) & ~63ull;
  if (cap < 64) cap = 64;
  if (cap > 4096) cap = 4096;
  return (uint32_t)cap;
}

void launch_emit(hipStream_t s, Grid g, Lattice lat, int kind, bool all_points, double alpha,
                 const double *sigma, const uint32_t *n_pts, const double *calc,
                 const unsigned long long *off, OutRows out, uint64_t rows_hint, int ewma_emit, uint32_t ewma_emit_rows) {
  if (g.K == 0) return;
  if (coop_shape(g)) {
    const int cblocks = (int)((g.K * 64 + kBlock - 1) / kBlock);
#define TAD_LAUNCH_EMIT_C(KIND, ALL) \
  hipLaunchKernelGGL((k_emit<KIND, ALL, true>), dim3(cblocks), dim3(kBlock), 0, s, g, lat, alpha, sigma, n_pts, calc, off, out)
    if (all_points) {
      if (kind == 0) TAD_LAUNCH_EMIT_C(0, true); else if (kind == 1) TAD_LAUNCH_EMIT_C(1, true); else if (kind == 3) TAD_LAUNCH_EMIT_C(3, true); else TAD_LAUNCH_EMIT_C(2, true);
    } else {
      if (kind == 0) TAD_LAUNCH_EMIT_C(0, false); else if (kind == 1) TAD_LAUNCH_EMIT_C(1, false); else if (kind == 3) TAD_LAUNCH_EMIT_C(3, false);
      else if (kind == 4) TAD_LAUNCH_EMIT_C(4, false); else TAD_LAUNCH_EMIT_C(2, false);
    }
#undef TAD_LAUNCH_EMIT_C
    return;
  }
  if (kind == 0 && !all_points && g.T < (1ull << kStageMarkTBits)) {
    if (const uint32_t cap = emit_stage_rows(g.K, rows_hint, ewma_emit, ewma_emit_rows)) {
      const unsigned blocks64 = (unsigned)((g.K + 63) / 64);
      hipLaunchKernelGGL(k_emit_staged, dim3(blocks64), dim3(64), (size_t)cap * 12 + 64 * 8, s, g, lat, alpha, sigma, n_pts, off, out, cap);
      return;
    }
  }
  const int blocks = (int)((g.K + kBlock - 1) / kBlock);
#define TAD_LAUNCH_EMIT(KIND, ALL) \
  hipLaunchKernelGGL((k_emit<KIND, ALL>), dim3(blocks), dim3(kBlock), 0, s, g, lat, alpha, sigma, n_pts, calc, off, out)
  if (all_points) {
    if (kind == 0) TAD_LAUNCH_EMIT(0, true); else if (kind == 1) TAD_LAUNCH_EMIT(1, true); else if (kind == 3) TAD_LAUNCH_EMIT(3, true); else TAD_LAUNCH_EMIT(2, true);
  } else {
    if (kind == 0) TAD_LAUNCH_EMIT(0, false); else if (kind == 1) TAD_LAUNCH_EMIT(1, false); else if (kind == 3) TAD_LAUNCH_EMIT(3, false);
    else if (kind == 4) TAD_LAUNCH_EMIT(4, false); else TAD_LAUNCH_EMIT(2, false);
  }
#undef TAD_LAUNCH_EMIT
}

__global__ __launch_bounds__(kBlock) void k_emit_points(Grid g, Lattice L, const unsigned long long *__restrict__ off,
                                                        unsigned long long *__restrict__ out_key, long long *__restrict__ out_t,
                                                        unsigned long long *__restrict__ out_val) {
  const uint64_t k = (uint64_t)blockIdx.x * kBlock + threadIdx.x;
  if (k >= g.K) return;
  unsigned long long pos = off[k];
  const unsigned long long end = off[k + 1];
  auto step = [&](uint64_t t, uint8_t fl, unsigned long long raw) {
    if ((fl & FLAG_PRESENT) && pos < end) {
      out_key[pos] = k;
      out_t[pos] = g.times != nullptr ? g.times[t * g.K + k] : (long long)(L.t0 + (int64_t)t * L.step);
      out_val[pos] = raw;
      pos++;
    }
  };
  uint64_t t = 0;
  for (; t + kUnroll <= g.T && pos < end; t += kUnroll) {
    uint8_t fl[kUnroll];
    unsigned long long v[kUnroll];
#pragma unroll
    for (int u = 0; u < kUnroll; ++u) { fl[u] = g.flag[(t + u) * g.K + k]; v[u] = g.val[(t + u) * g.K + k]; }
#pragma unroll
    for (int u = 0; u < kUnroll; ++u) step(t + u, fl[u], v[u]);
  }
  for (; t < g.T && pos < end; ++t) step(t, g.flag[t * g.K + k], g.val[t * g.K + k]);
}

void launch_emit_points(hipStream_t s, Grid g, Lattice lat, const unsigned long long *off, unsigned long long *out_key,
                        long long *out_t, unsigned long long *out_val) {
  if (g.K == 0) return;
  const int blocks = (int)((g.K + kBlock - 1) / kBlock);
  hipLaunchKernelGGL(k_emit_points, dim3(blocks), dim3(kBlock), 0, s, g, lat, off, out_key, out_t, out_val);
}


__device__ __forceinline__ void stream_row(OutRows out, unsigned long long pos, uint64_t k, long long ts, double x, double e, double sg,
                                           bool all, bool verdict) {
  out.key_id[pos] = k;
  out.flow_end_s[pos] = ts;
  out.throughput[pos] = x;
  out.algo_calc[pos] = e;
  out.stddev[pos] = sg;
  if (all) out.anomaly[pos] = verdict ? 1 : 0;
}

__device__ __forceinline__ void stream_counters(unsigned long long my_pts, unsigned my_key, uint32_t err, DevCounters *ctr) {
  for (int d = 32; d >= 1; d >>= 1) {
    my_pts += __shfl_down(my_pts, d);
    my_key += __shfl_down(my_key, d);
    err |= __shfl_down(err, d);
  }
  if ((threadIdx.x & 63) == 0) {
    if (my_key) { atomicAdd(&ctr->n_points, my_pts); atomicAdd(&ctr->n_keys, (unsigned long long)my_key); }
    if (err) atomicOr(&ctr->err, err);
  }
}

template <bool EMIT, bool ALL>
__global__ __launch_bounds__(kBlock) void k_stream(Grid g, Lattice L, double alpha, StreamState cur, StreamState next,
                                                   uint32_t *__restrict__ n_anom, const unsigned long long *__restrict__ off,
                                                   OutRows out, DevCounters *ctr) {
  const uint64_t k = (uint64_t)blockIdx.x * kBlock + threadIdx.x;
  unsigned long long my_pts = 0;
  unsigned my_key = 0;
  uint32_t err = 0;
  if (k < g.K) {
    StreamAcc st = stream_load(cur, k);
    const double one_minus = 1.0 - alpha;
    unsigned long long pos = EMIT ? off[k] : 0ull;
    uint32_t a = 0, fresh = 0;
    walk_series(g, k, [&](uint64_t t, uint8_t fl, unsigned long long raw) {
      if (!(fl & FLAG_PRESENT)) return;
// ... 106 lines not shown
```

theia_amd/csrc/tad_stage0_part.hip:

```cpp
#include <cstdlib>
#include <cstring>

#include "tad_internal.h"

namespace tad {

static constexpr int kPartThreads = 1024;

static constexpr int kMinCellBits = 15, kMaxCellBits = 24;
static constexpr uint32_t kTileCells = 17744;
static constexpr uint32_t kMaxParts = 2048;
static constexpr size_t kLdsBudget = 156 * 1024;
static constexpr int kGcdSamples = 4;

__device__ __forceinline__ void lds_barrier() { asm volatile("s_waitcnt lgkmcnt(0)\n\ts_barrier" ::: "memory"); }

__device__ __forceinline__ uint64_t p_gcd_u64(uint64_t a, uint64_t b) {
  if (a == 0) return b;
  if (b == 0) return a;
  if (((a | b) >> 32) == 0) {
    uint32_t x = (uint32_t)a, y = (uint32_t)b;
    while (y) { uint32_t r = x % y; x = y; y = r; }
    return x;
  }
// ... 837 lines not shown
              uint32_t sl = 0;
              if (srank == 0) sl = atomicAdd(&s_nspill, (uint32_t)__popcll(spl));
              sl = (uint32_t)__shfl((int)sl, (int)__builtin_ctzll(spl)) + srank;
#else
              const uint32_t sl = atomicAdd(&s_nspill, 1u);
#endif
              if (sl < kSpillSlots) { s_spill_rec[sl] = rec; s_spill_at[sl] = at; }
              else A.recs[at] = rec;
            } else err |= DEV_ERR_REGION_FULL;
          }
        } else if (kept && k != TAD_KEY_SKIP) {
          err |= DEV_ERR_KEY_RANGE;
        }
      }
    }
    load_tile(r, tile + 2);
    lds_barrier();
    const uint32_t nj = s_njobs;
    for (uint32_t j = threadIdx.x / SEC; j < nj; j += kPartThreads / SEC) {
      const uint32_t p = jobs[j], sl = threadIdx.x & (SEC - 1u);
      const uint32_t word = cnt[p], qo = word >> 16, qcap = (cnt[p + 1] >> 16) - qo;
      const uint32_t c0 = word & 0xFFFFu, c = c0 < qcap ? c0 : qcap, g = gcur[p];
      unsigned long long *qp = q + qo;
      const uint32_t whole = c & ~(uint32_t)(SEC - 1);
      const uint32_t room = gend[p] - g, sp = nsp[p];
      const bool fits = sp <= room && whole <= room - sp;
      if (fits) { for (uint32_t o = 0; o < whole; o += SEC) A.recs[g + o + sl] = qp[o + sl]; }
      else err |= DEV_ERR_REGION_FULL;
      const bool mv = whole + sl < c;
      const unsigned long long tail = mv ? qp[whole + sl] : 0ull;
      if (mv) qp[sl] = tail;
      if (sl == 0) { cnt[p] = (qo << 16) | (c - whole); gcur[p] = g + whole; }
    }
    {
      const uint32_t ns = s_nspill < kSpillSlots ? s_nspill : kSpillSlots;
      for (uint32_t i = threadIdx.x; i < ns; i += kPartThreads) A.recs[s_spill_at[i]] = s_spill_rec[i];
    }
    lds_barrier();
    if (threadIdx.x == 0) { s_njobs = 0; s_nspill = 0; }
  };

  Rows R0, R1;
  load_tile(R0, 0);
  load_tile(R1, 1);
  lds_barrier();
  for (uint64_t tile = 0; tile < ntiles; tile += 2) {
    process(R0, tile);
    if (tile + 1 < ntiles) process(R1, tile + 1);
  }
  for (uint32_t p = threadIdx.x; p < F; p += kPartThreads) {
    const uint32_t word = cnt[p], qo = word >> 16, qcap = (cnt[p + 1] >> 16) - qo;
    const uint32_t c = (word & 0xFFFFu) < qcap ? (word & 0xFFFFu) : qcap;
    uint32_t g = gcur[p];
    const uint32_t room = gend[p] - g;
    const uint32_t e = gend[p] - (nsp[p] < room ? nsp[p] : room);
    if (A.fin != nullptr) {
      if (c <= e - g && g <= e) { for (uint32_t i = 0; i < c; ++i) A.recs[g + i] = q[qo + i]; g += c; }
      else err |= DEV_ERR_REGION_FULL;
      uint32_t *fo = A.fin + ((size_t)blockIdx.x * F + p) * 2;
      fo[0] = g; fo[1] = e;
    } else if (c <= e - g && g <= e) {
      for (uint32_t i = 0; i < c; ++i) A.recs[g + i] = q[qo + i];
      for (g += c; g < e; ++g) A.recs[g] = ~0ull;
    } else {
      err |= DEV_ERR_REGION_FULL;
    }
  }
  block_count_rows(used, err, A.ctr);
}

static constexpr uint32_t kSliceRecords = 1u << 17;

struct TileGeom {
  int shift_part;
  int cell_bits;
  uint32_t nparts;
  uint32_t tb;
  uint32_t n_chunks;
  uint32_t par_rounds;
  uint32_t slice_len;
  uint32_t kt;
};

template <bool OPMAX, bool SETTLE, bool NARROW>
__device__ __forceinline__ void tile_aggregate_body(const unsigned long long *__restrict__ recs,
                                                    const unsigned long long *__restrict__ part_start,
                                                    SliceTable st, TileGeom tg, Grid g,
                                                    const uint32_t *__restrict__ offs32, const uint32_t *__restrict__ fin, int G,
                                                    SettleArgs sa, const unsigned long long *__restrict__ ovf_count_in) {
  uint32_t s_idx = blockIdx.x, r_lo = 0, r_hi = tg.n_chunks;
  if (tg.par_rounds && tg.n_chunks > 1) {
    const uint32_t x = blockIdx.x & 7u, y = blockIdx.x >> 3;
    r_lo = y % tg.n_chunks;
    r_hi = r_lo + 1;
    s_idx = (y / tg.n_chunks) * 8u + x;
  }
  if (s_idx >= *st.n_slices) return;
  const uint32_t p = st.slice_part[s_idx];
  const uint32_t first = st.slice_first[p];
  const uint32_t nsl = (p + 1 < tg.nparts ? st.slice_first[p + 1] : *st.n_slices) - first;
  const bool split = nsl > 1;
  const int shift_part = tg.shift_part;
  const uint32_t KP = 1u << shift_part;
  const uint32_t T = (uint32_t)g.T;
  const uint64_t k0 = (uint64_t)p << shift_part;
  extern __shared__ __attribute__((aligned(16))) unsigned char smem[];
  __shared__ uint32_t s_nlist, s_lbase, s_nredo, s_rbase;
  __shared__ uint32_t s_ovfw[40];
  const uint32_t cell_none = (1u << tg.cell_bits) - 1u;
  const unsigned long long plo = part_start[p], phi = part_start[p + 1];
  const unsigned long long lo = plo + (unsigned long long)(s_idx - first) * tg.slice_len;
  const unsigned long long hi = lo + tg.slice_len < phi ? lo + tg.slice_len : phi;
  for (uint32_t chunk = r_lo; chunk < r_hi; ++chunk) {
    const uint32_t KT = SETTLE ? tg.kt : KP;
    const uint32_t kt0 = SETTLE ? chunk * KT : 0u;
    const uint32_t b_lo = SETTLE ? 0u : chunk * tg.tb;
    const uint32_t nb = SETTLE ? T : (b_lo + tg.tb <= T ? tg.tb : T - b_lo);
    const uint32_t cells = SETTLE ? nb * KT : nb << shift_part;
    const uint32_t c_lo = b_lo << shift_part;
    unsigned long long *vals = reinterpret_cast<unsigned long long *>(smem);
    uint32_t *vals32 = reinterpret_cast<uint32_t *>(smem);
    uint8_t *flags = smem + (size_t)(SETTLE ? tg.tb * KT : tg.tb << shift_part) * (NARROW ? 4 : 8);
    auto cell_present = [&](uint32_t c) -> bool { return NARROW ? vals32[c] != 0u : (flags[c] & FLAG_PRESENT) != 0; };
    auto cell_value = [&](uint32_t c) -> unsigned long long { return NARROW ? (unsigned long long)(vals32[c] - 1u) : vals[c]; };
    if (chunk != r_lo) __syncthreads();
    if (NARROW) {
      for (uint32_t c = threadIdx.x; c < cells; c += kPartThreads) vals32[c] = 0u;
    } else {
      for (uint32_t c = threadIdx.x; c < cells; c += kPartThreads) vals[c] = 0ull;
      for (uint32_t c = threadIdx.x; c < (cells + 3) / 4; c += kPartThreads) reinterpret_cast<uint32_t *>(flags)[c] = 0u;
    }
    __syncthreads();
    auto apply = [&](unsigned long long r) {
      const uint32_t cg = (uint32_t)r & cell_none;
      uint32_t c = cg - c_lo;
      if (SETTLE) {
        const uint32_t kk = (cg & (KP - 1u)) - kt0;
        if (cg == cell_none || kk >= KT) return;
        c = __umul24(cg >> shift_part, KT) + kk;
      } else if (c >= cells) return;
      const unsigned long long v = r >> tg.cell_bits;
      if (NARROW) { atomicMax(&vals32[c], (uint32_t)v + 1u); return; }
      if (OPMAX) atomicMax(&vals[c], v);
      else atomicAdd(&vals[c], v);
      flags[c] = FLAG_PRESENT;
    };
    constexpr int U = 8;
    uint32_t ovf_w = 0;
    const uint64_t ovf_k0 = (k0 + (SETTLE ? chunk * tg.kt : 0u)) & ~(uint64_t)31;
    if (SETTLE && sa.ovf_keys != nullptr && threadIdx.x < 40u) {
      const uint64_t wi = (ovf_k0 >> 5) + threadIdx.x;
      if (wi < (g.K + 31) / 32) ovf_w = sa.ovf_keys[wi];
    }
    if (fin != nullptr) {
      const uint32_t wave = threadIdx.x >> 6, lane = threadIdx.x & 63u;
      const uint32_t F = tg.nparts;
      for (uint32_t w0 = wave; w0 < (uint32_t)G; w0 += 64u * (kPartThreads / 64)) {
        const uint32_t wm = w0 + lane * (kPartThreads / 64);
        unsigned long long b_start = 0, b_lo = 0, b_hi = 0, b_end = 0;
        if (wm < (uint32_t)G) {
          b_start = plo + offs32[(size_t)wm * F + p];
          b_end = wm + 1 < (uint32_t)G ? plo + offs32[(size_t)(wm + 1) * F + p] : phi;
          b_lo = fin[((size_t)wm * F + p) * 2];
          b_hi = fin[((size_t)wm * F + p) * 2 + 1];
        }
        for (uint32_t j = 0; j < 64u && w0 + j * (kPartThreads / 64) < (uint32_t)G; ++j) {
          const unsigned long long r_start = __shfl(b_start, (int)j), r_lo = __shfl(b_lo, (int)j), r_hi = __shfl(b_hi, (int)j),
// ... 84 lines not shown
            s1 = as1 + (bs1 + dnb * sh);
            s2 = as2 + (bs2 + 2.0 * sh * bs1 + dnb * (sh * sh));
          }
        }
        if (part != 0 || kk >= KT) continue;
        if (!live) { settled[kk] = 1; continue; }
        const bool key_ovf = sa.ovf_keys != nullptr && ((s_ovfw[(uint32_t)((k - ovf_k0) >> 5)] >> (k & 31u)) & 1u) != 0;
        if (!skip_cols || key_ovf) { sa.st.n_pts[k] = kSettleRedo; settled[kk] = 0; tile_redo[atomicAdd(&s_nredo, 1u)] = (uint32_t)k; continue; }
        const bool slow = n > 0 && (!(mx - mn <= sa.eps) || n < (uint32_t)sa.min_samples);
        sa.st.n_pts[k] = n;
        sa.st.n_anom[k] = 0;
        const double dn = (double)(n ? n : 1);
        sa.st.key_mean[k] = n ? x0 + s1 / dn : 0.0;
        sa.st.key_m2[k] = n ? fmax(s2 - s1 * (s1 / dn), 0.0) : 0.0;
        settled[kk] = slow ? 0 : 1;
        if (slow) tile_list[atomicAdd(&s_nlist, 1u)] = (uint32_t)k;
      }
      __syncthreads();
      if (threadIdx.x == 0 && s_nlist) s_lbase = atomicAdd(sa.count, s_nlist);
      if (threadIdx.x == 64 && s_nredo) s_rbase = atomicAdd(sa.redo_count, s_nredo);
      __syncthreads();
      for (uint32_t i = threadIdx.x; i < s_nlist; i += kPartThreads) sa.list[s_lbase + i] = tile_list[i];
      for (uint32_t i = threadIdx.x; i < s_nredo; i += kPartThreads) sa.redo_list[s_rbase + i] = tile_redo[i];
      if (sa.rs_val != nullptr && s_nredo) {
        const uint32_t wave = threadIdx.x >> 6, lane = threadIdx.x & 63u;
        for (uint32_t i = wave; i < s_nredo; i += kPartThreads / 64) {
          const uint32_t e = s_rbase + i;
          if (e >= sa.rs_cap) continue;
          if (skip_cols) {
            const uint32_t kk = tile_redo[i] - (uint32_t)(k0 + kt0);
            for (uint32_t b = lane; b < nb; b += 64) {
              const uint32_t c = __umul24(b, KT) + kk;
              const bool pr = cell_present(c);
              sa.rs_val[(size_t)e * nb + b] = pr ? cell_value(c) : 0ull;
              sa.rs_flag[(size_t)e * nb + b] = pr ? (uint8_t)(FLAG_PRESENT | ((NARROW && vals32[c] == 0xFFFFFFFFu) ? 2 : 0)) : 0;
            }
          }
          if (lane == 0) sa.rs_has[e] = skip_cols ? (NARROW ? 1 : 2) : 0;
        }
      }
      if (sa.cs_val != nullptr) {
        const uint32_t wave = threadIdx.x >> 6, lane = threadIdx.x & 63u;
        for (uint32_t i = wave; i < s_nlist; i += kPartThreads / 64) {
          const uint32_t e = s_lbase + i;
          if (e >= sa.cs_cap) continue;
          const uint32_t kk = tile_list[i] - (uint32_t)(k0 + kt0);
          for (uint32_t b = lane; b < nb; b += 64) {
            const uint32_t c = __umul24(b, KT) + kk;
            const bool pr = cell_present(c);
            sa.cs_val[(size_t)e * nb + b] = pr ? cell_value(c) : 0ull;
            sa.cs_flag[(size_t)e * nb + b] = pr ? FLAG_PRESENT : 0;
          }
          if (lane == 0) sa.cs_has[e] = 1;
        }
      }
    }
    if (SETTLE) {
      for (uint32_t kk = threadIdx.x & 255u; kk < KT; kk += 256u) {
        const uint64_t k = k0 + kt0 + kk;
        if (kt0 + kk < KP && k < g.K && !(skip_cols && settled[kk])) {
          for (uint32_t b = threadIdx.x >> 8; b < nb; b += kPartThreads / 256) {
            const uint32_t c = __umul24(b, KT) + kk;
            const uint64_t gc = (uint64_t)b * g.K + k;
            const bool pr = cell_present(c);
            const unsigned long long cv = pr ? cell_value(c) : 0ull;
            if (!split) {
              g.val[gc] = cv;
              g.flag[gc] = pr ? FLAG_PRESENT : 0;
            } else if (pr) {
              if (OPMAX) __hip_atomic_fetch_max(g.val + gc, cv, __ATOMIC_RELAXED, __HIP_MEMORY_SCOPE_AGENT);
              else __hip_atomic_fetch_add(g.val + gc, cv, __ATOMIC_RELAXED, __HIP_MEMORY_SCOPE_AGENT);
              g.flag[gc] = FLAG_PRESENT;
            }
          }
        }
      }
    } else {
      for (uint32_t c = threadIdx.x; c < cells; c += kPartThreads) {
        const uint32_t b = b_lo + (c >> shift_part), kk = c & (KP - 1);
        const uint64_t k = k0 + kk;
        if (k >= g.K) continue;
        const uint64_t gc = (uint64_t)b * g.K + k;
        if (!split) {
          g.val[gc] = vals[c];
          g.flag[gc] = flags[c];
        } else if (flags[c]) {
          if (OPMAX) __hip_atomic_fetch_max(g.val + gc, vals[c], __ATOMIC_RELAXED, __HIP_MEMORY_SCOPE_AGENT);
          else __hip_atomic_fetch_add(g.val + gc, vals[c], __ATOMIC_RELAXED, __HIP_MEMORY_SCOPE_AGENT);
          g.flag[gc] = FLAG_PRESENT;
        }
      }
    }
  }
}

template <bool OPMAX, bool SETTLE = false, bool NARROW = false>
__global__ __launch_bounds__(kPartThreads) void k_tile_aggregate(const unsigned long long *__restrict__ recs,
                                                                 const unsigned long long *__restrict__ part_start,
                                                                 SliceTable st, TileGeom tg, Grid g,
                                                                 const uint32_t *__restrict__ offs32, const uint32_t *__restrict__ fin, int G,
                                                                 SettleArgs sa, const unsigned long long *__restrict__ ovf_count) {
  static_assert(!NARROW || (OPMAX && SETTLE), "32-bit tile cells: settle mode with max only");
  tile_aggregate_body<OPMAX, SETTLE, NARROW>(recs, part_start, st, tg, g, offs32, fin, G, sa, ovf_count);
}

template <bool OPMAX>
__global__ __launch_bounds__(256) void k_apply_overflow(const OverflowRec *__restrict__ ovf,
                                                        const unsigned long long *__restrict__ ovf_count, uint32_t cap, Grid g) {
  unsigned long long n = *ovf_count;
  if (n > cap) n = cap;
  for (unsigned long long i = (unsigned long long)blockIdx.x * 256 + threadIdx.x; i < n; i += (unsigned long long)gridDim.x * 256) {
    const OverflowRec r = ovf[i];
    if (OPMAX) __hip_atomic_fetch_max(g.val + r.gcell, r.val, __ATOMIC_RELAXED, __HIP_MEMORY_SCOPE_AGENT);
    else __hip_atomic_fetch_add(g.val + r.gcell, r.val, __ATOMIC_RELAXED, __HIP_MEMORY_SCOPE_AGENT);
    g.flag[r.gcell] = FLAG_PRESENT;
  }
}



bool part_plan_bins(uint64_t n, uint64_t K, bool has2, PartPlan *pl) {
  if (K == 0 || n == 0 || n * (has2 ? 2 : 1) >= (1ull << 32)) return false;
  int s = 0;
  while (((K + (1ull << s) - 1) >> s) > kMaxBins) ++s;
  pl->shift_bin = s;
  pl->nbins = (uint32_t)((K + (1ull << s) - 1) >> s);
  pl->G = 256;
  uint64_t chunk = (n + pl->G - 1) / pl->G;
  chunk = (chunk + 1) & ~1ull;
  pl->chunk = chunk;
  return true;
}

bool part_plan_tiles(uint64_t K, uint64_t T, bool has2, PartPlan *pl) {
  if (T == 0 || T >= (1ull << 16)) return false;
  int sp_fit = -1;
  for (int c = 13; c >= 0; --c)
    if (((uint64_t)T << c) <= kTileCells) { sp_fit = c; break; }
  int sp = sp_fit >= pl->shift_bin ? sp_fit : pl->shift_bin;
  while (((K + (1ull << sp) - 1) >> sp) > kMaxParts && sp < 13) ++sp;
  if (((K + (1ull << sp) - 1) >> sp) > kMaxParts) return false;
  while (sp > pl->shift_bin && (1ull << (sp - 1)) >= K) --sp;
  {
    auto parts_of = [&](int c) { return (K + (1ull << c) - 1) >> c; };
    auto rounds_of = [&](int c) { const uint64_t tb = kTileCells >> c; return tb ? (T + tb - 1) / tb : (uint64_t)1 << 30; };
    const uint64_t line_parts = kLdsBudget / (8 * 18 + 18);
    if (parts_of(sp) > line_parts) {
      int c = sp;
      while (c < 13 && parts_of(c) > line_parts) ++c;
      if (parts_of(c) <= line_parts && (1ull << c) <= kTileCells && rounds_of(c) <= 2 * rounds_of(sp) && rounds_of(c) <= 4) sp = c;
    }
  }
  {
    auto parts_of = [&](int c) { return (K + (1ull << c) - 1) >> c; };
    auto rounds_of = [&](int c) { const uint64_t tb = kTileCells >> c; return tb ? (T + tb - 1) / tb : (uint64_t)1 << 30; };
    const uint64_t sector_parts = kLdsBudget / (8 * 9 + 18);
    if (parts_of(sp) > sector_parts && sp < 13 && parts_of(sp + 1) <= sector_parts && (1ull << (sp + 1)) <= kTileCells && rounds_of(sp + 1) <= 8) ++sp;
  }
  if ((1ull << sp) > kTileCells) return false;
  pl->shift_part = sp;
  pl->KP = 1u << sp;
  pl->nparts = (uint32_t)((K + pl->KP - 1) >> sp);
  pl->bins_per_part = 1u << (sp - pl->shift_bin);
  const uint64_t cells_all = (uint64_t)pl->KP * T;
  int cb = kMinCellBits;
  while (cb < kMaxCellBits && (1ull << cb) - 1 <= cells_all) ++cb;
  if ((1ull << cb) - 1 <= cells_all) return false;
  pl->cell_bits = cb;
  pl->tb = (uint32_t)(kTileCells >> sp);
  if (pl->tb > T) pl->tb = (uint32_t)T;
  pl->n_chunks = (uint32_t)((T + pl->tb - 1) / pl->tb);
  pl->tb = (uint32_t)((T + pl->n_chunks - 1) / pl->n_chunks);
  pl->agg_lds = ((size_t)pl->tb * pl->KP * 9 + 15) & ~(size_t)15;
  const size_t fixed = ((size_t)pl->nparts + 4) * 16 + 64;
  pl->rpt = 0;
  const int mult = has2 ? 2 : 1;
  for (int r : {10, 8, 4, 2}) {
    const size_t slots = (size_t)r * kPartThreads * mult;
    if (slots * 10 + fixed <= kLdsBudget) { pl->rpt = r; pl->part_lds = (slots * 10 + fixed + 15) & ~(size_t)15; break; }
  }
  return pl->rpt != 0;
}

bool part_plan_sparse(uint64_t K, uint64_t T, bool has2, PartPlan *pl) {
  (void)has2;
  if (T == 0 || T >= (1ull << 32) || K == 0) return false;
  int tbits = 0;
  while ((T >> tbits) != 0) ++tbits;
  auto parts_of = [&](int c) { return (K + (1ull << c) - 1) >> c; };
  const uint64_t sector_parts = kLdsBudget / (8 * 9 + 18);
  int sp = pl->shift_bin;
  while (sp < 13 && parts_of(sp) > sector_parts) ++sp;
// ... 118 lines not shown
  A.round_mask = sampled ? 15u : (pl.wc_cap ? pl.wc_sec - 1u : 0u);
  A.G = pl.G; A.partials = sampled ? partials : nullptr; A.n = n; A.chunk = pl.chunk;
  A.offs32 = offs32; A.total = total; A.part_start = part_start;
  A.st = slice_table(slice_mem, slots, pl);
  A.slice_len = g.val == nullptr ? 0xFFFFFFFFu : slice_len_of(sampled, slots, pl.nparts);
  A.g = g; A.shift_part = pl.shift_part; A.ctr = sampled ? ctr : nullptr;
  hipLaunchKernelGGL(k_part_offsets, dim3((pl.nparts + 3) / 4), dim3(256), 0, s, A);
  hipLaunchKernelGGL(k_part_tail, dim3(1), dim3(256), 0, s, A);
}

void launch_partition(hipStream_t s, const uint64_t *key, const uint64_t *key2, const int64_t *t_end,
                      const int64_t *t_start, const uint64_t *value, uint64_t n, uint64_t K, RowFilter f, Lattice L,
                      const PartPlan &pl, const uint32_t *offs32, const unsigned long long *part_start, void *recs,
                      OverflowRec *ovf, unsigned long long *ovf_count, uint32_t ovf_cap, DevCounters *ctr, uint32_t *fin, uint32_t *ovf_keys, int cw) {
  PartArgs A;
  A.fin = fin; A.G = pl.G;
  A.value_limit = 1ull << (64 - pl.cell_bits);
  A.narrow_limit = pl.narrow ? 0xFFFFFFFEull : 0ull;
  A.ovf_keys = ovf_keys;
  A.key = key; A.key2 = key2; A.t_end = t_end; A.t_start = t_start; A.value = value;
  A.n = n; A.chunk = pl.chunk; A.K = K; A.f = f; A.L = L;
  A.shift_part = pl.shift_part; A.kp_mask = pl.KP - 1; A.nparts = pl.nparts; A.cell_bits = pl.cell_bits;
  A.offs32 = offs32; A.part_start = part_start;
  A.recs = static_cast<unsigned long long *>(recs); A.ctr = ctr;
  A.ovf = ovf; A.ovf_count = ovf_count; A.ovf_cap = ovf_cap;
  const bool has2 = key2 != nullptr;
  const bool vec = aligned16(key) && aligned16(key2) && aligned16(t_end) && aligned16(value);
  const bool generic = !vec || L.mode == 2 || f.end_time != 0 || (f.start_time != 0 && t_start != nullptr);
  with_widths(cw, [&](auto k32, auto t32) {
    constexpr bool K32 = decltype(k32)::value, T32 = decltype(t32)::value;
    if (pl.wc_cap) {
      const size_t wlds = ((size_t)pl.nparts * (8 * (size_t)pl.wc_cap + kWcFixedBytes) + 4 + 15) & ~(size_t)15;
      const bool ts16 = generic && t_start != nullptr && f.start_time != 0 && aligned16(t_start);
#define TAD_WC1(RPT, SEC, H2, GEN, TS)                                                                                  \
  do {                                                                                                                \
    allow_big_lds(reinterpret_cast<const void *>(k_partition_wc<RPT, SEC, H2, GEN, TS, K32, T32>), kLdsBudget);        \
    hipLaunchKernelGGL((k_partition_wc<RPT, SEC, H2, GEN, TS, K32, T32>), dim3(pl.G), dim3(kPartThreads), wlds, s, A, pl.wc_cap, pl.G); \
  } while (0)
#define TAD_WC(RPT, SEC, H2, GEN) do { if (GEN && ts16) TAD_WC1(RPT, SEC, H2, GEN, GEN); else TAD_WC1(RPT, SEC, H2, GEN, false); } while (0)
#define TAD_WC_SEC(RPT, H2, GEN) do { if (pl.wc_sec == 16) TAD_WC(RPT, 16, H2, GEN); else TAD_WC(RPT, 8, H2, GEN); } while (0)
      if (pl.wc_rpt == 4 && !has2) { if (generic) TAD_WC_SEC(4, false, true); else TAD_WC_SEC(4, false, false); }
      else if (has2) { if (generic) TAD_WC_SEC(2, true, true); else TAD_WC_SEC(2, true, false); }
      else { if (generic) TAD_WC_SEC(2, false, true); else TAD_WC_SEC(2, false, false); }
#undef TAD_WC_SEC
#undef TAD_WC
#undef TAD_WC1
      return;
    }
    int rpt = pl.rpt;
    if (generic && rpt > 4) rpt = 4;
    if ((K32 || T32) && rpt > 4) rpt = 4;
    const size_t fixed = ((size_t)pl.nparts + 4) * 16 + 64;
    const size_t lds = ((size_t)rpt * kPartThreads * (has2 ? 2 : 1) * 10 + fixed + 15) & ~(size_t)15;
#define TAD_PART(RPT, H2, V, GEN)                                                                                       \
  do {                                                                                                                \
    allow_big_lds(reinterpret_cast<const void *>(k_partition<RPT, H2, V, GEN, K32, T32>), kLdsBudget);                 \
    hipLaunchKernelGGL((k_partition<RPT, H2, V, GEN, K32, T32>), dim3(pl.G), dim3(kPartThreads), lds, s, A);            \
  } while (0)
    if (!generic) {
      switch (rpt) {
        case 10: if constexpr (!K32 && !T32) { if (has2) TAD_PART(8, true, true, false); else TAD_PART(10, false, true, false); } break;
        case 8: if constexpr (!K32 && !T32) { if (has2) TAD_PART(8, true, true, false); else TAD_PART(8, false, true, false); } break;
        case 6: case 4: if (has2) TAD_PART(4, true, true, false); else TAD_PART(4, false, true, false); break;
        default: if (has2) TAD_PART(2, true, true, false); else TAD_PART(2, false, true, false); break;
      }
    } else if (vec) {
      if (rpt >= 4) { if (has2) TAD_PART(4, true, true, true); else TAD_PART(4, false, true, true); }
      else { if (has2) TAD_PART(2, true, true, true); else TAD_PART(2, false, true, true); }
    } else {
      if (rpt >= 4) { if (has2) TAD_PART(4, true, false, true); else TAD_PART(4, false, false, true); }
      else { if (has2) TAD_PART(2, true, false, true); else TAD_PART(2, false, false, true); }
    }
#undef TAD_PART
  });
}

size_t slice_table_bytes(uint64_t slots, const PartPlan &pl) {
  const size_t max_slices = (size_t)pl.nparts + (size_t)(slots / kSliceRecords) + 1;
  return (max_slices + pl.nparts + 4) * sizeof(uint32_t);
}

void launch_tile_aggregate(hipStream_t s, const void *recs, const unsigned long long *part_start, const PartPlan &pl,
                           uint64_t slots, void *slice_mem, Grid g, bool op_max, const OverflowRec *ovf,
                           const unsigned long long *ovf_count, uint32_t ovf_cap, const uint32_t *offs32, const uint32_t *fin, SettleArgs settle) {
  const unsigned long long *rr = static_cast<const unsigned long long *>(recs);
  const uint32_t max_slices = (uint32_t)((size_t)pl.nparts + (size_t)(slots / kSliceRecords) + 1);
  const SliceTable st = slice_table(slice_mem, slots, pl);
  const uint32_t slice_len = slice_len_of(fin != nullptr, slots, pl.nparts);
  const uint32_t par = pl.n_chunks > 1 ? 1u : 0u;
  const bool settle_on = settle.on != 0 && pl.settle_kt != 0;
  TileGeom tg{pl.shift_part, pl.cell_bits, pl.nparts, pl.tb, pl.n_chunks, par, slice_len, settle_on ? pl.settle_kt : 0u};
  const uint32_t blocks1 = par ? ((max_slices + 7u) / 8u) * 8u * pl.n_chunks : max_slices;
  const SettleArgs none{};
#define TAD_TA(OPMAX, SET)                                                                                                                            \
  do {                                                                                                                                               \
    allow_big_lds(reinterpret_cast<const void *>(k_tile_aggregate<OPMAX, SET>), kLdsBudget);                                                         \
    hipLaunchKernelGGL((k_tile_aggregate<OPMAX, SET>), dim3(blocks1), dim3(kPartThreads), pl.agg_lds, s, rr, part_start, st, tg, g, offs32, fin, pl.G, \
                       SET ? settle : none, ovf_count);                                                                                               \
    hipLaunchKernelGGL((k_apply_overflow<OPMAX>), dim3(64), dim3(256), 0, s, ovf, ovf_count, ovf_cap, g);                                             \
  } while (0)
  if (settle_on && pl.narrow && op_max) {
    allow_big_lds(reinterpret_cast<const void *>(k_tile_aggregate<true, true, true>), kLdsBudget);
    hipLaunchKernelGGL((k_tile_aggregate<true, true, true>), dim3(blocks1), dim3(kPartThreads), pl.agg_lds, s, rr, part_start, st, tg, g, offs32, fin, pl.G, settle, ovf_count);
    hipLaunchKernelGGL((k_apply_overflow<true>), dim3(64), dim3(256), 0, s, ovf, ovf_count, ovf_cap, g);
  } else if (settle_on) { if (op_max) TAD_TA(true, true); else TAD_TA(false, true); }
  else { if (op_max) TAD_TA(true, false); else TAD_TA(false, false); }
#undef TAD_TA
}

const void *code_anchor_stage0_part() { return reinterpret_cast<const void *>(&k_part_tail); }

}
```

Before: 77.65 billion.

## Store EWMA grid cells as packed f64 with sign-encoded absence

New measurement: 78.07 billion (median of 6 runs). Within noise of the previous version (+0.6%).

```diff
diff --git a/theia_amd/csrc/tad_capi.cpp b/theia_amd/csrc/tad_capi.cpp
--- a/theia_amd/csrc/tad_capi.cpp
+++ b/theia_amd/csrc/tad_capi.cpp
@@ -41,7 +41,7 @@
     return;
   launch_emit(e->stream, g, L, kind, jp.all_points, jp.alpha, static_cast<const double *>(e->sigma.p),
               static_cast<const uint32_t *>(e->n_pts.p), static_cast<const double *>(kind == 3 ? e->key_mean.p : e->calc.p),
-              static_cast<const unsigned long long *>(e->off.p), out, rows, e->plan.ewma_emit, e->plan.ewma_emit_rows);
+              static_cast<const unsigned long long *>(e->off.p), out, rows, e->plan.ewma_emit, e->plan.ewma_emit_rows, jp.f64_grid);
 }
 
 int make_result(JobCtx *e, uint64_t rows, bool with_anomaly, tad_mem out_memory, ResultPriv **out, OutRows *dev_rows,
diff --git a/theia_amd/csrc/tad_capi_job.cpp b/theia_amd/csrc/tad_capi_job.cpp
--- a/theia_amd/csrc/tad_capi_job.cpp
+++ b/theia_amd/csrc/tad_capi_job.cpp
@@ -36,6 +36,9 @@
   const uint32_t *binhist = nullptr;
   const unsigned long long *stream_poff = nullptr;
   uint64_t stream_P = 0;
+  uint64_t tile_slots = 0;
+  const uint32_t *tile_fin = nullptr;
+  int extra_syncs = 0;
   int stage0_path() const { return sparse ? (sp_part ? 8 : 4) : (v2 ? (pl.wc_cap ? 3 : 2) : 1); }
   int hist_source() const { return (v2 && hist_sampled) ? 1 : (use_kh ? 2 : 0); }
 };
@@ -76,7 +79,7 @@
                 static_cast<double *>(e->key_mean.p), static_cast<double *>(e->key_m2.p), ctr);
   } else if (!db_fused)
     launch_key_sigma(s, g, jp.alpha, ewma && !jp.all_points, static_cast<const double *>(e->rcp_table.p), sigma, n_pts, n_anom, ctr, static_cast<double *>(e->key_mean.p),
-                     static_cast<double *>(e->key_m2.p));
+                     static_cast<double *>(e->key_m2.p), jp.f64_grid);
   if (jp.algo == TAD_ALGO_DBSCAN) {
     if ((rc = ensure(e, e->aux, dbscan_scratch_bytes(g))) != TAD_OK) return rc;
     if (dbscan_uses_list(g)) {
@@ -443,13 +446,27 @@
   SettleArgs settle;
   uint32_t *ovf_keys;
   if ((rc = settle_setup(e, j, rs, a, &settle, &ovf_keys)) != TAD_OK) return rc;
+  j.jp.f64_grid = j.jp.algo == TAD_ALGO_EWMA && !j.jp.all_points && !j.points_mode && !j.stream && grid_f64_shape(a.g);
+  a.tile_slots = slots;
+  a.tile_fin = fin;
   HIP_TRY(e, hipEventRecord(e->ev[2], s));
   launch_partition(s, (const uint64_t *)j.d_key, (const uint64_t *)j.d_key2, (const int64_t *)j.d_te, (const int64_t *)j.d_ts,
                    (const uint64_t *)j.d_val, n, K, j.rf, a.L, pl, offs32, part_start, e->recs.p, ovf, ovf_count, kOverflowCap, j.ctr, fin, ovf_keys, j.cw);
   HIP_TRY(e, hipEventRecord(e->ev[3], s));
   launch_tile_aggregate(s, e->recs.p, part_start, pl, slots, e->slices.p, a.g, j.op_max, ovf, ovf_count, kOverflowCap,
-                        a.hist_sampled ? offs32 : nullptr, fin, settle);
-  return TAD_OK;
+                        a.hist_sampled ? offs32 : nullptr, fin, settle, j.jp.f64_grid);
+  return TAD_OK;
+}
+
+int rerun_integer_grid(JobCtx *e, Job &j, Attempt &a, uint64_t *rows) {
+  hipStream_t s = e->stream;
+  j.jp.f64_grid = false;
+  a.extra_syncs++;
+  HIP_TRY(e, hipMemsetAsync(&j.ctr->n_keys, 0, 2 * sizeof(unsigned long long), s));
+  launch_tile_aggregate(s, e->recs.p, static_cast<const unsigned long long *>(e->part_start.p), a.pl, a.tile_slots, e->slices.p, a.g, j.op_max,
+                        reinterpret_cast<const OverflowRec *>(static_cast<unsigned char *>(e->ovf.p) + 16), dev_ovf_count(e), kOverflowCap,
+                        a.hist_sampled ? static_cast<const uint32_t *>(e->part_offs32.p) : nullptr, a.tile_fin, SettleArgs{}, false);
+  return detect_and_count(e, a.g, j.jp, j.ctr, rows);
 }
 
 int stage0_dense(JobCtx *e, Job &j, Stage0Retry &rs, Attempt &a) {
@@ -681,7 +698,7 @@
   if ((rc = finish_rows(e, j.job, &ro, rows, jp.all_points, c, g.K != 0)) != TAD_OK) return rc;
   tad_stats &st = ro.rp->pub.stats;
   stage0_stats(e, j, a, c, attempts, st);
-  st.host_syncs = (a.hinted || j.empty) ? 2 : 3;
+  st.host_syncs = ((a.hinted || j.empty) ? 2 : 3) + a.extra_syncs;
   if (stream && g.K) {
     unsigned long long added = 0;
     memcpy(&added, e->tail_host + kTailHistLen, 8);
@@ -730,6 +747,7 @@
     Attempt a;
     HIP_TRY(e, hipMemsetAsync(j.ctr, 0, kTailMoments, s));
     j.jp.settled = false;
+    j.jp.f64_grid = false;
     if ((rc = derive_lattice(e, j, rs, a)) != TAD_OK) return rc;
     if (a.retry) continue;
     if ((rc = choose_stage0(e, j, rs, a)) != TAD_OK) return rc;
@@ -744,7 +762,12 @@
     StreamBatches sb;
     if (j.points_mode) rc = count_points(e, j, a, &rows);
     else if (stream) rc = count_stream(e, j, a, &sb, &rows);
-    else rc = detect_and_count(e, a.g, j.jp, j.ctr, &rows);
+    else {
+      rc = detect_and_count(e, a.g, j.jp, j.ctr, &rows);
+      unsigned long long ovf_n = 0;
+      memcpy(&ovf_n, e->tail_host + kTailOvfCount, 8);
+      if (rc == TAD_OK && j.jp.f64_grid && ovf_n != 0) rc = rerun_integer_grid(e, j, a, &rows);
+    }
     if (rc != TAD_OK) return rc;
     const DevCounters c = *e->ctr_host;
     if ((rc = decide(e, j, rs, a, c.err)) != TAD_OK) return rc;
diff --git a/theia_amd/csrc/tad_engine.h b/theia_amd/csrc/tad_engine.h
--- a/theia_amd/csrc/tad_engine.h
+++ b/theia_amd/csrc/tad_engine.h
@@ -301,6 +301,7 @@
   bool all_points;
   bool lazy_sigma = false;
   bool settled = false;
+  bool f64_grid = false;
 };
 
 int ensure_rcp_table(JobCtx *e, uint64_t T);
diff --git a/theia_amd/csrc/tad_internal.h b/theia_amd/csrc/tad_internal.h
--- a/theia_amd/csrc/tad_internal.h
+++ b/theia_amd/csrc/tad_internal.h
@@ -25,6 +25,8 @@
 };
 
 enum : uint8_t { FLAG_PRESENT = 1, FLAG_ANOMALY = 2 };
+
+static constexpr unsigned long long kF64Absent = 0xBFF0000000000000ull;
 
 struct MetaPartial {
   int64_t tmin, tmax, tref;
@@ -142,6 +144,35 @@
     }
   }
   for (uint64_t t = nfull * kWalkChunk; t < T; ++t) step(t, g.flag[t * g.K + k], g.val[t * g.K + k]);
+}
+
+template <typename Step>
+__device__ __forceinline__ void walk_series_f64(const Grid &g, uint64_t k, Step step) {
+  const uint64_t T = g.T;
+  const uint64_t nfull = T / kWalkChunk;
+  unsigned long long va[kWalkChunk], vb[kWalkChunk];
+  auto load = [&](uint64_t c, unsigned long long *v) {
+#pragma unroll
+    for (int u = 0; u < kWalkChunk; ++u) v[u] = g.val[(c * kWalkChunk + u) * g.K + k];
+  };
+  auto one = [&](uint64_t t, unsigned long long w) { step(t, (int32_t)(w >> 32) >= 0, __longlong_as_double((long long)w)); };
+  if (nfull) {
+    load(0, va);
+    uint64_t c = 0;
+    for (; c + 2 <= nfull; c += 2) {
+      load(c + 1, vb);
+#pragma unroll
+      for (int u = 0; u < kWalkChunk; ++u) one(c * kWalkChunk + u, va[u]);
+      load(c + 2 < nfull ? c + 2 : c + 1, va);
+#pragma unroll
+      for (int u = 0; u < kWalkChunk; ++u) one((c + 1) * kWalkChunk + u, vb[u]);
+    }
+    if (c < nfull) {
+#pragma unroll
+      for (int u = 0; u < kWalkChunk; ++u) one(c * kWalkChunk + u, va[u]);
+    }
+  }
+  for (uint64_t t = nfull * kWalkChunk; t < T; ++t) one(t, g.val[t * g.K + k]);
 }
 
 static constexpr uint64_t kCoopMinT = 512, kCoopMaxK = 8192;
@@ -199,7 +230,7 @@
 #endif
 
 void launch_key_sigma(hipStream_t s, Grid g, double alpha, bool ewma_count, const double *rcp, double *sigma,
-                      uint32_t *n_pts, uint32_t *n_anom, DevCounters *ctr, double *key_mean, double *key_m2);
+                      uint32_t *n_pts, uint32_t *n_anom, DevCounters *ctr, double *key_mean, double *key_m2, bool f64 = false);
 static constexpr int kMomentBlocks = 128;
 void launch_moments(hipStream_t s, uint64_t K, const uint32_t *n_pts, const double *key_mean,
                     const double *key_m2, Moments *partials, DevCounters *ctr = nullptr);
@@ -213,7 +244,8 @@
 void launch_emit(hipStream_t s, Grid g, Lattice lat, int kind, bool all_points, double alpha,
                  const double *sigma, const uint32_t *n_pts, const double *calc,
                  const unsigned long long *off, OutRows out, uint64_t rows_hint = 0,
-                 int ewma_emit = 0, uint32_t ewma_emit_rows = 0);
+                 int ewma_emit = 0, uint32_t ewma_emit_rows = 0,
+                 bool f64 = false);
 void launch_emit_points(hipStream_t s, Grid g, Lattice lat, const unsigned long long *off, unsigned long long *out_key,
                         long long *out_t, unsigned long long *out_val);
 struct StreamState {
@@ -470,7 +502,9 @@
 size_t slice_table_bytes(uint64_t slots, const PartPlan &pl);
 void launch_tile_aggregate(hipStream_t s, const void *recs, const unsigned long long *part_start, const PartPlan &pl,
                            uint64_t slots, void *slice_mem, Grid g, bool op_max, const OverflowRec *ovf,
-                           const unsigned long long *ovf_count, uint32_t ovf_cap, const uint32_t *offs32, const uint32_t *fin, SettleArgs settle);
+                           const unsigned long long *ovf_count, uint32_t ovf_cap, const uint32_t *offs32, const uint32_t *fin, SettleArgs settle,
+                           bool f64 = false);
+bool grid_f64_shape(Grid g);
 bool part_plan_settle(uint64_t T, PartPlan *pl, bool narrow = false);
 
 size_t sparse_sort_temp_bytes(uint64_t slots);
diff --git a/theia_amd/csrc/tad_kernels.hip b/theia_amd/csrc/tad_kernels.hip
--- a/theia_amd/csrc/tad_kernels.hip
+++ b/theia_amd/csrc/tad_kernels.hip
@@ -209,11 +209,12 @@
 
 static constexpr int kUnroll = 16;
 
-template <bool EWMA_COUNT, bool RCP_LDS, bool COOP = false>
+template <bool EWMA_COUNT, bool RCP_LDS, bool COOP = false, bool F64 = false>
 __global__ __launch_bounds__(kBlock) void k_key_sigma(Grid g, double alpha, const double *__restrict__ rcp_g, double *__restrict__ sigma,
                                                       uint32_t *__restrict__ n_pts,
                                                       uint32_t *__restrict__ n_anom, DevCounters *ctr,
                                                       double *__restrict__ key_mean, double *__restrict__ key_m2) {
+  static_assert(!F64 || !COOP, "F64 cells: lane-per-key walks only");
   const uint64_t gtid = (uint64_t)blockIdx.x * kBlock + threadIdx.x;
   const uint64_t k = COOP ? gtid >> 6 : gtid;
   const bool writer = !COOP || (threadIdx.x & 63) == 0;
@@ -253,6 +254,17 @@
                          avg = avg + dn;
                          m2 = m2 + d * (d - dn);
                        });
+    } else if constexpr (F64) {
+      walk_series_f64(g, k, [&](uint64_t, bool present, double x) {
+        if (present) {
+          cnt = cnt + 1.0;
+          n++;
+          const double d = x - avg;
+          const double dn = RCP_LDS ? div_by_count(d, cnt, rcp[n]) : d / cnt;
+          avg = avg + dn;
+          m2 = m2 + d * (d - dn);
+        }
+      });
     } else {
       walk_series(g, k, sigma_step);
     }
@@ -281,6 +293,12 @@
                     e = one_minus * e + alpha * x;
                     a += fabs(x - e) > sg ? 1u : 0u;
                   });
+        else if constexpr (F64) walk_series_f64(g, k, [&](uint64_t, bool present, double x) {
+                    if (present) {
+                      e = one_minus * e + alpha * x;
+                      a += fabs(x - e) > sg ? 1u : 0u;
+                    }
+                  });
         else walk_series(g, k, ewma_step);
       }
       if (writer) n_anom[k] = a;
@@ -296,11 +314,21 @@
   }
 }
 
+bool grid_f64_shape(Grid g) { return g.times == nullptr && !coop_shape(g); }
+
 void launch_key_sigma(hipStream_t s, Grid g, double alpha, bool ewma_count, const double *rcp, double *sigma,
-                      uint32_t *n_pts, uint32_t *n_anom, DevCounters *ctr, double *key_mean, double *key_m2) {
+                      uint32_t *n_pts, uint32_t *n_anom, DevCounters *ctr, double *key_mean, double *key_m2, bool f64) {
   if (g.K == 0) return;
   const size_t lds = (size_t)(g.T + 1) * 8;
   const bool in_lds = lds <= 32768;
+  if (f64) {
+    if (!ewma_count || !grid_f64_shape(g)) abort();
+    const int blocks = (int)((g.K + kBlock - 1) / kBlock);
+#define TAD_KSF(RL) hipLaunchKernelGGL((k_key_sigma<true, RL, false, true>), dim3(blocks), dim3(kBlock), RL ? lds : 0, s, g, alpha, rcp, sigma, n_pts, n_anom, ctr, key_mean, key_m2)
+    if (in_lds) TAD_KSF(true); else TAD_KSF(false);
+#undef TAD_KSF
+    return;
+  }
   if (coop_shape(g)) {
     const int cblocks = (int)((g.K * 64 + kBlock - 1) / kBlock);
 #define TAD_KSC(EC, RL) hipLaunchKernelGGL((k_key_sigma<EC, RL, true>), dim3(cblocks), dim3(kBlock), RL ? lds : 0, s, g, alpha, rcp, sigma, n_pts, n_anom, ctr, key_mean, key_m2)
@@ -540,7 +568,7 @@
   scan_launches(s, cnt, off, K, scratch, total_copy, &M);
 }
 
-template <int KIND, bool ALL, bool COOP = false>
+template <int KIND, bool ALL, bool COOP = false, bool F64 = false>
 __global__ __launch_bounds__(kBlock) void k_emit(Grid g, Lattice L, double alpha,
                                                  const double *__restrict__ sigma,
                                                  const uint32_t *__restrict__ n_pts,
@@ -623,7 +651,9 @@
       }
     }
   };
+  static_assert(!F64 || (KIND == 0 && !ALL && !COOP), "F64 cells: the EWMA job's lane-per-key emit only");
   if (COOP) walk_series_coop(g, k, [](uint64_t) {}, [&](uint64_t t, uint8_t fl, double x, int) { point(t, fl, x); });
+  else if constexpr (F64) walk_series_f64(g, k, [&](uint64_t t, bool present, double x) { if (present) point(t, FLAG_PRESENT, x); });
   else walk_series(g, k, [&](uint64_t t, uint8_t fl, unsigned long long raw) { if (fl & FLAG_PRESENT) point(t, fl, (double)raw); });
 #pragma unroll
   for (int i = 0; i < 3; ++i)
@@ -636,6 +666,7 @@
 }
 
 static constexpr int kStageMarkTBits = 26;
+template <bool F64 = false>
 __global__ __launch_bounds__(64) void k_emit_staged(Grid g, Lattice L, double alpha, const double *__restrict__ sigma,
                                                     const uint32_t *__restrict__ n_pts,
                                                     const unsigned long long *__restrict__ off, OutRows out, uint32_t cap) {
@@ -658,9 +689,7 @@
   if (pos != end) {
     const double one_minus = 1.0 - alpha;
     double e = 0.0;
-    walk_series(g, k, [&](uint64_t t, uint8_t fl, unsigned long long raw) {
-      if (!(fl & FLAG_PRESENT)) return;
-      const double x = (double)raw;
+    auto point = [&](uint64_t t, double x) {
       e = one_minus * e + alpha * x;
       if (fabs(x - e) > sg && pos < end) {
         if (pos < cap) {
@@ -676,7 +705,9 @@
         }
         pos++;
       }
-    });
+    };
+    if constexpr (F64) walk_series_f64(g, k, [&](uint64_t t, bool present, double x) { if (present) point(t, x); });
+    else walk_series(g, k, [&](uint64_t t, uint8_t fl, unsigned long long raw) { if (fl & FLAG_PRESENT) point(t, (double)raw); });
   }
   __syncthreads();
   const unsigned long long staged = total < cap ? total : cap;
@@ -688,7 +719,7 @@
     const unsigned long long at = base + r;
     out.key_id[at] = k0 + ln;
     out.flow_end_s[at] = g.times != nullptr ? g.times[cell] : (long long)(L.t0 + (int64_t)t * L.step);
-    out.throughput[at] = (double)g.val[cell];
+    out.throughput[at] = F64 ? __longlong_as_double((long long)g.val[cell]) : (double)g.val[cell];
     out.algo_calc[at] = s_e[r];
     out.stddev[at] = s_sg[ln];
   }
@@ -710,8 +741,9 @@
 
 void launch_emit(hipStream_t s, Grid g, Lattice lat, int kind, bool all_points, double alpha,
                  const double *sigma, const uint32_t *n_pts, const double *calc,
-                 const unsigned long long *off, OutRows out, uint64_t rows_hint, int ewma_emit, uint32_t ewma_emit_rows) {
+                 const unsigned long long *off, OutRows out, uint64_t rows_hint, int ewma_emit, uint32_t ewma_emit_rows, bool f64) {
   if (g.K == 0) return;
+  if (f64 && !(kind == 0 && !all_points && grid_f64_shape(g))) abort();
   if (coop_shape(g)) {
     const int cblocks = (int)((g.K * 64 + kBlock - 1) / kBlock);
 #define TAD_LAUNCH_EMIT_C(KIND, ALL) \
@@ -728,11 +760,16 @@
   if (kind == 0 && !all_points && g.T < (1ull << kStageMarkTBits)) {
     if (const uint32_t cap = emit_stage_rows(g.K, rows_hint, ewma_emit, ewma_emit_rows)) {
       const unsigned blocks64 = (unsigned)((g.K + 63) / 64);
-      hipLaunchKernelGGL(k_emit_staged, dim3(blocks64), dim3(64), (size_t)cap * 12 + 64 * 8, s, g, lat, alpha, sigma, n_pts, off, out, cap);
+      if (f64) hipLaunchKernelGGL(k_emit_staged<true>, dim3(blocks64), dim3(64), (size_t)cap * 12 + 64 * 8, s, g, lat, alpha, sigma, n_pts, off, out, cap);
+      else hipLaunchKernelGGL(k_emit_staged<false>, dim3(blocks64), dim3(64), (size_t)cap * 12 + 64 * 8, s, g, lat, alpha, sigma, n_pts, off, out, cap);
       return;
     }
   }
   const int blocks = (int)((g.K + kBlock - 1) / kBlock);
+  if (f64) {
+    hipLaunchKernelGGL((k_emit<0, false, false, true>), dim3(blocks), dim3(kBlock), 0, s, g, lat, alpha, sigma, n_pts, calc, off, out);
+    return;
+  }
 #define TAD_LAUNCH_EMIT(KIND, ALL) \
   hipLaunchKernelGGL((k_emit<KIND, ALL>), dim3(blocks), dim3(kBlock), 0, s, g, lat, alpha, sigma, n_pts, calc, off, out)
   if (all_points) {
diff --git a/theia_amd/csrc/tad_stage0_part.hip b/theia_amd/csrc/tad_stage0_part.hip
--- a/theia_amd/csrc/tad_stage0_part.hip
+++ b/theia_amd/csrc/tad_stage0_part.hip
@@ -943,7 +943,7 @@
   uint32_t kt;
 };
 
-template <bool OPMAX, bool SETTLE, bool NARROW>
+template <bool OPMAX, bool SETTLE, bool NARROW, bool F64>
 __device__ __forceinline__ void tile_aggregate_body(const unsigned long long *__restrict__ recs,
                                                     const unsigned long long *__restrict__ part_start,
                                                     SliceTable st, TileGeom tg, Grid g,
@@ -1194,8 +1194,12 @@
         if (k >= g.K) continue;
         const uint64_t gc = (uint64_t)b * g.K + k;
         if (!split) {
-          g.val[gc] = vals[c];
-          g.flag[gc] = flags[c];
+          if constexpr (F64) {
+            g.val[gc] = flags[c] ? (unsigned long long)__double_as_longlong((double)vals[c]) : kF64Absent;
+          } else {
+            g.val[gc] = vals[c];
+            g.flag[gc] = flags[c];
+          }
         } else if (flags[c]) {
           if (OPMAX) __hip_atomic_fetch_max(g.val + gc, vals[c], __ATOMIC_RELAXED, __HIP_MEMORY_SCOPE_AGENT);
           else __hip_atomic_fetch_add(g.val + gc, vals[c], __ATOMIC_RELAXED, __HIP_MEMORY_SCOPE_AGENT);
@@ -1206,20 +1210,48 @@
   }
 }
 
-template <bool OPMAX, bool SETTLE = false, bool NARROW = false>
+template <bool OPMAX, bool SETTLE = false, bool NARROW = false, bool F64 = false>
 __global__ __launch_bounds__(kPartThreads) void k_tile_aggregate(const unsigned long long *__restrict__ recs,
                                                                  const unsigned long long *__restrict__ part_start,
                                                                  SliceTable st, TileGeom tg, Grid g,
                                                                  const uint32_t *__restrict__ offs32, const uint32_t *__restrict__ fin, int G,
                                                                  SettleArgs sa, const unsigned long long *__restrict__ ovf_count) {
   static_assert(!NARROW || (OPMAX && SETTLE), "32-bit tile cells: settle mode with max only");
-  tile_aggregate_body<OPMAX, SETTLE, NARROW>(recs, part_start, st, tg, g, offs32, fin, G, sa, ovf_count);
-}
-
-template <bool OPMAX>
+  static_assert(!F64 || !SETTLE, "F64 cells: the EWMA job, no settle mode");
+  tile_aggregate_body<OPMAX, SETTLE, NARROW, F64>(recs, part_start, st, tg, g, offs32, fin, G, sa, ovf_count);
+}
+
+template <bool OPMAX, bool F64 = false>
 __global__ __launch_bounds__(256) void k_apply_overflow(const OverflowRec *__restrict__ ovf,
-                                                        const unsigned long long *__restrict__ ovf_count, uint32_t cap, Grid g) {
+                                                        const unsigned long long *__restrict__ ovf_count, uint32_t cap, Grid g,
+                                                        SliceTable st, uint32_t nparts, int shift_part) {
   unsigned long long n = *ovf_count;
+  if constexpr (F64) {
+    __shared__ uint32_t s_split[kMaxParts];
+    __shared__ uint32_t s_nsplit;
+    if (threadIdx.x == 0) s_nsplit = 0;
+    __syncthreads();
+    const uint32_t ns = *st.n_slices;
+    for (uint32_t p = threadIdx.x; p < nparts && p < kMaxParts; p += 256u) {
+      const uint32_t first = st.slice_first[p];
+      const uint32_t next = p + 1 < nparts ? st.slice_first[p + 1] : ns;
+      if (first < ns && next <= ns && next > first + 1u) s_split[atomicAdd(&s_nsplit, 1u)] = p;
+    }
+    __syncthreads();
+    const uint32_t KP = 1u << shift_part;
+    const uint64_t cells_all = (uint64_t)KP * g.T;
+    for (uint32_t j = 0; j < s_nsplit; ++j) {
+      const uint64_t k0 = (uint64_t)s_split[j] << shift_part;
+      for (uint64_t c = (uint64_t)blockIdx.x * 256 + threadIdx.x; c < cells_all; c += (uint64_t)gridDim.x * 256) {
+        const uint64_t b = c >> shift_part, k = k0 + (c & (KP - 1));
+        if (k >= g.K) continue;
+        const uint64_t gc = b * g.K + k;
+        if (n == 0) g.val[gc] = (g.flag[gc] & FLAG_PRESENT) ? (unsigned long long)__double_as_longlong((double)g.val[gc]) : kF64Absent;
+        else { g.val[gc] = 0ull; g.flag[gc] = 0; }
+      }
+    }
+    return;
+  }
   if (n > cap) n = cap;
   for (unsigned long long i = (unsigned long long)blockIdx.x * 256 + threadIdx.x; i < n; i += (unsigned long long)gridDim.x * 256) {
     const OverflowRec r = ovf[i];
@@ -1504,7 +1536,8 @@
 
 void launch_tile_aggregate(hipStream_t s, const void *recs, const unsigned long long *part_start, const PartPlan &pl,
                            uint64_t slots, void *slice_mem, Grid g, bool op_max, const OverflowRec *ovf,
-                           const unsigned long long *ovf_count, uint32_t ovf_cap, const uint32_t *offs32, const uint32_t *fin, SettleArgs settle) {
+                           const unsigned long long *ovf_count, uint32_t ovf_cap, const uint32_t *offs32, const uint32_t *fin, SettleArgs settle,
+                           bool f64) {
   const unsigned long long *rr = static_cast<const unsigned long long *>(recs);
   const uint32_t max_slices = (uint32_t)((size_t)pl.nparts + (size_t)(slots / kSliceRecords) + 1);
   const SliceTable st = slice_table(slice_mem, slots, pl);
@@ -1519,15 +1552,28 @@
     allow_big_lds(reinterpret_cast<const void *>(k_tile_aggregate<OPMAX, SET>), kLdsBudget);                                                         \
     hipLaunchKernelGGL((k_tile_aggregate<OPMAX, SET>), dim3(blocks1), dim3(kPartThreads), pl.agg_lds, s, rr, part_start, st, tg, g, offs32, fin, pl.G, \
                        SET ? settle : none, ovf_count);                                                                                               \
-    hipLaunchKernelGGL((k_apply_overflow<OPMAX>), dim3(64), dim3(256), 0, s, ovf, ovf_count, ovf_cap, g);                                             \
+    hipLaunchKernelGGL((k_apply_overflow<OPMAX>), dim3(64), dim3(256), 0, s, ovf, ovf_count, ovf_cap, g, st, pl.nparts, pl.shift_part);              \
   } while (0)
+#define TAD_TA_F64(OPMAX)                                                                                                                             \
+  do {                                                                                                                                               \
+    allow_big_lds(reinterpret_cast<const void *>(k_tile_aggregate<OPMAX, false, false, true>), kLdsBudget);                                          \
+    hipLaunchKernelGGL((k_tile_aggregate<OPMAX, false, false, true>), dim3(blocks1), dim3(kPartThreads), pl.agg_lds, s, rr, part_start, st, tg, g,   \
+                       offs32, fin, pl.G, none, ovf_count);                                                                                          \
+    hipLaunchKernelGGL((k_apply_overflow<OPMAX, true>), dim3(64), dim3(256), 0, s, ovf, ovf_count, ovf_cap, g, st, pl.nparts, pl.shift_part);       \
+  } while (0)
+  if (f64) {
+    if (settle_on) abort();
+    if (op_max) TAD_TA_F64(true); else TAD_TA_F64(false);
+    return;
+  }
   if (settle_on && pl.narrow && op_max) {
     allow_big_lds(reinterpret_cast<const void *>(k_tile_aggregate<true, true, true>), kLdsBudget);
     hipLaunchKernelGGL((k_tile_aggregate<true, true, true>), dim3(blocks1), dim3(kPartThreads), pl.agg_lds, s, rr, part_start, st, tg, g, offs32, fin, pl.G, settle, ovf_count);
-    hipLaunchKernelGGL((k_apply_overflow<true>), dim3(64), dim3(256), 0, s, ovf, ovf_count, ovf_cap, g);
+    hipLaunchKernelGGL((k_apply_overflow<true>), dim3(64), dim3(256), 0, s, ovf, ovf_count, ovf_cap, g, st, pl.nparts, pl.shift_part);
   } else if (settle_on) { if (op_max) TAD_TA(true, true); else TAD_TA(false, true); }
   else { if (op_max) TAD_TA(true, false); else TAD_TA(false, false); }
 #undef TAD_TA
+#undef TAD_TA_F64
 }
 
 const void *code_anchor_stage0_part() { return reinterpret_cast<const void *>(&k_part_tail); }
```
